# mrazomej/BarBay.jl

Measured on AMD Instinct MI355X. Metric: ELBO-grad steps/sec, 50k barcodes x 8 timepoints, higher is better.
Workload: dtype f64

## Files before the change

### barbay.jl_amd/_capi.py

```python
from __future__ import annotations

import ctypes as C
import os
from typing import Dict, List, Optional, Sequence, Tuple

import numpy as np

_HERE = os.path.dirname(os.path.abspath(__file__))
LIB_PATH = os.path.join(_HERE, "lib", "libbarbay_hip.so")

BB_MODEL = {"fitness": 0, "multienv": 1, "genotype": 2, "replicate": 3, "multienv_replicate": 4}
BB_OPT_TRUNCATED_ADAGRAD = 0
BB_OPT_DECAYED_ADAGRAD = 1
BB_COMM_ID_BYTES = 128
BB_P2P_HANDLE_BYTES = 64
BB_LOGP_MAX_BATCH = 64
BB_CHAIN_MAX_K = 16384
BB_CHAIN_MAX_Q = 8
BB_CHAIN_LAG_BATCH = 32
BB_TRACE_MAX_SNAPSHOTS = 16384
BB_SCORE_MAX_SAMPLES = 16384
BB_RB_MAX_SAMPLES = 8672
BB_RB_MAX_Q = 8
BB_THETA_RB_CHUNK = 64
BB_POPMEAN_RB_CHUNK = 256
BB_MATH_FN = {"exp": 0, "log": 1, "rcp": 2, "div": 3, "sqrt": 4, "softplus_sigmoid": 5, "sincospi": 6, "exp_nonpos": 7, "log_1to2": 8,
              "box_muller": 9}
BB_ERR_UNSUPPORTED = -4
BB_ERR_NONFINITE = -5

EXPORTS = [
    "bb_version", "bb_last_error", "bb_default_opts", "bb_create", "bb_destroy", "bb_num_latents",
    "bb_get_layout", "bb_init_meanfield", "bb_set_params", "bb_get_params", "bb_get_permutation", "bb_get_owned", "bb_run", "bb_run_profiled",
    "bb_get_posterior", "bb_elbo_grad", "bb_logdensity_grad", "bb_logdensity_grad_batch", "bb_get_elbo_trace", "bb_debug_normals", "bb_debug_math", "bb_debug_stamps", "bb_debug_graph_launches", "bb_get_stats", "bb_kernel_name",
    "bb_comm_make_id", "bb_comm_init", "bb_step_moments", "bb_step_apply", "bb_hier_units", "bb_hier_fitness", "bb_p2p_export", "bb_p2p_import", "bb_p2p_selftest", "bb_p2p_enable",
    "bb_ppc_shape", "bb_ppc_bands", "bb_freq_shape", "bb_freq_bands", "bb_score_shape", "bb_ppc_score", "bb_chain_summary",
    "bb_fitness_rb_shape", "bb_fitness_rb", "bb_theta_rb_shape", "bb_theta_rb", "bb_popmean_rb_shape", "bb_popmean_rb",
    "bb_trace_begin", "bb_trace_end", "bb_trace_count", "bb_trace_get", "bb_trace_summary",
]

_dp = C.POINTER(C.c_double)


class bb_prior(C.Structure):
    _fields_ = [("mean", _dp), ("std", _dp), ("n", C.c_int64)]


class bb_model_desc(C.Structure):
    _fields_ = [
        ("kind", C.c_int32), ("n_rep", C.c_int32), ("n_neutral", C.c_int64), ("n_bc", C.c_int64),
        ("n_time", C.POINTER(C.c_int32)), ("counts", C.POINTER(C.c_int64)), ("totals", C.POINTER(C.c_int64)),
        ("n_env", C.c_int32), ("env_idx", C.POINTER(C.c_int32)),
        ("n_geno", C.c_int32), ("geno_idx", C.POINTER(C.c_int32)),
        ("s_pop_prior", bb_prior), ("logsigma_pop_prior", bb_prior), ("s_bc_prior", bb_prior),
        ("logsigma_bc_prior", bb_prior), ("loglambda_prior", bb_prior), ("logtau_prior", bb_prior),
        ("flags", C.c_int32),
    ]


class bb_advi_opts(C.Structure):
    _fields_ = [
        ("samples_per_step", C.c_int32), ("optimizer", C.c_int32), ("eta", C.c_double), ("tau", C.c_double),
        ("window", C.c_int32), ("resum_every", C.c_int32), ("pre", C.c_double), ("post", C.c_double),
        ("seed", C.c_uint64), ("device", C.c_int32), ("rank", C.c_int32), ("world_size", C.c_int32),
        ("steps_per_graph", C.c_int32), ("elbo_every", C.c_int32), ("launch_mode", C.c_int32),
        ("n_devices", C.c_int32), ("device_ids", C.POINTER(C.c_int32)),
    ]


class bb_block_range(C.Structure):
    _fields_ = [("name", C.c_char * 24), ("lo", C.c_int64), ("hi", C.c_int64)]


class bb_stats(C.Structure):
    _fields_ = [
        ("n_latents", C.c_int64), ("n_moments", C.c_int64), ("steps_done", C.c_int64),
        ("shard_lo", C.c_int64), ("shard_hi", C.c_int64), ("bytes_per_step", C.c_int64),
        ("bytes_sample", C.c_int64), ("bytes_update", C.c_int64), ("last_run_ms", C.c_double),
        ("avg_sample_ms", C.c_double), ("avg_update_ms", C.c_double),
        ("n_blocks", C.c_int32), ("block_threads", C.c_int32), ("lds_bytes", C.c_int32),
        ("persistent_pairs", C.c_int32), ("launches_last_run", C.c_int32), ("resident_kernel", C.c_int32),
        ("geno_lo", C.c_int32), ("geno_hi", C.c_int32),
        ("device_bytes", C.c_int64), ("window_row", C.c_int64),
        ("rows_same_xcd", C.c_int32), ("reserved0", C.c_int32),
    ]


class bb_ppc_opts(C.Structure):
    _fields_ = [
        ("n_samples", C.c_int32), ("n_ppc", C.c_int32), ("n_quantiles", C.c_int32), ("reserved0", C.c_int32),
        ("quantiles", _dp), ("seed", C.c_uint64),
    ]


BB_FREQ_MODE = {"trajectory": 0, "posterior": 1}


class bb_freq_opts(C.Structure):
    _fields_ = [
        ("mode", C.c_int32), ("n_samples", C.c_int32), ("n_ppc", C.c_int32), ("n_quantiles", C.c_int32),
        ("quantiles", _dp), ("seed", C.c_uint64),
    ]


class bb_score_opts(C.Structure):
    _fields_ = [("n_samples", C.c_int32), ("reserved0", C.c_int32), ("seed", C.c_uint64)]


SCORE_CELLS = ("observed", "pred_mean", "pred_sd", "lpd", "p_waic", "pit", "pit_upper")
SCORE_ROWS = ("row_lpd", "row_p_waic")


class bb_score_out(C.Structure):
    _fields_ = [(k, _dp) for k in SCORE_CELLS + SCORE_ROWS] + [("n_scored", C.POINTER(C.c_int32))]


RB_UNITS = ("q_mean", "q_sd", "rb_mean", "rb_sd", "p_pos", "p_neg")


class bb_rb_opts(C.Structure):
    _fields_ = [("n_samples", C.c_int32), ("n_quantiles", C.c_int32), ("probs", _dp), ("threshold", C.c_double), ("seed", C.c_uint64),
                ("draws", _dp)]


class bb_rb_out(C.Structure):
    _fields_ = [(k, _dp) for k in RB_UNITS] + [("quantiles", _dp), ("n_steps", C.POINTER(C.c_int32))]


class bb_theta_rb_out(C.Structure):
    _fields_ = [(k, _dp) for k in RB_UNITS] + [("quantiles", _dp), ("n_members", C.POINTER(C.c_int32)), ("n_steps", C.POINTER(C.c_int32))]


class bb_popmean_rb_out(C.Structure):
    _fields_ = [(k, _dp) for k in RB_UNITS] + [("quantiles", _dp), ("n_members", C.POINTER(C.c_int32))]


class bb_chain_opts(C.Structure):
    _fields_ = [
        ("n_chains", C.c_int32), ("n_draws", C.c_int32), ("n_quantiles", C.c_int32), ("max_lag", C.c_int32),
        ("probs", _dp), ("slab_cols", C.c_int64),
    ]


class bb_chain_out(C.Structure):
    _fields_ = [
        ("mean", _dp), ("sd", _dp), ("mcse", _dp), ("ess", _dp), ("rhat", _dp), ("quantiles", _dp),
        ("n_lags", C.POINTER(C.c_int32)),
    ]


class bb_trace_opts(C.Structure):
    _fields_ = [("every", C.c_int32), ("capacity", C.c_int32)]


class bb_trace_sum_opts(C.Structure):
    _fields_ = [
        ("first", C.c_int64), ("n_chains", C.c_int32), ("n_draws", C.c_int32), ("max_lag", C.c_int32), ("reserved0", C.c_int32),
        ("slab_cols", C.c_int64), ("rhat_max", C.c_double),
    ]


TRACE_COLS = ("mean", "sd", "mcse", "ess", "rhat")
TRACE_BLOCK_COUNTS = ("n_cols", "n_nonfinite", "n_const", "n_above")
TRACE_BLOCK_VALUES = ("max_rhat", "min_ess", "max_mcse_rel")


class bb_trace_block(C.Structure):
    _fields_ = ([("name", C.c_char * 24), ("part", C.c_int32), ("reserved0", C.c_int32)] + [(k, C.c_int64) for k in TRACE_BLOCK_COUNTS]
                + [(k, C.c_double) for k in TRACE_BLOCK_VALUES])


class bb_trace_sum_out(C.Structure):
    _fields_ = [(k, _dp) for k in TRACE_COLS] + [("n_lags", C.POINTER(C.c_int32)), ("blocks", C.POINTER(bb_trace_block))]


class BarBayHipError(RuntimeError):
    """Raised for any non-zero status of the C ABI (the reference throws ErrorException)."""


class BarBayNonFinite(BarBayHipError):
    """bb_run took its steps but the variational parameters went NaN / Inf (BB_ERR_NONFINITE); the state can still be read."""


def _declare(lib: C.CDLL) -> C.CDLL:
    vp = C.c_void_p
    lib.bb_version.restype = C.c_char_p
    lib.bb_last_error.restype = C.c_char_p
    lib.bb_default_opts.argtypes = [C.POINTER(bb_advi_opts)]
    lib.bb_default_opts.restype = None
    lib.bb_create.argtypes = [C.POINTER(bb_model_desc), C.POINTER(bb_advi_opts), C.POINTER(vp)]
    lib.bb_destroy.argtypes = [vp]
    lib.bb_destroy.restype = None
    lib.bb_num_latents.argtypes = [vp]
    lib.bb_num_latents.restype = C.c_int64
    lib.bb_get_layout.argtypes = [vp, C.POINTER(bb_block_range), C.POINTER(C.c_int32)]
    lib.bb_init_meanfield.argtypes = [vp]
    lib.bb_set_params.argtypes = [vp, _dp, _dp]
    lib.bb_get_params.argtypes = [vp, _dp, _dp]
    if hasattr(lib, "bb_get_permutation"):
        lib.bb_get_permutation.argtypes = [vp, C.POINTER(C.c_int64)]
    if hasattr(lib, "bb_get_owned"):
        lib.bb_get_owned.argtypes = [vp, C.POINTER(C.c_int64), C.POINTER(C.c_int64)]
    lib.bb_run.argtypes = [vp, C.c_int64]
    lib.bb_run_profiled.argtypes = [vp, C.c_int64]
    lib.bb_get_posterior.argtypes = [vp, _dp, _dp]
    lib.bb_elbo_grad.argtypes = [vp, _dp, _dp, _dp, C.c_int32, _dp, _dp, _dp]
    lib.bb_logdensity_grad.argtypes = [vp, _dp, _dp, _dp]
    lib.bb_logdensity_grad_batch.argtypes = [vp, C.c_int32, _dp, _dp, _dp]
    lib.bb_get_elbo_trace.argtypes = [vp, C.c_int64, C.c_int64, _dp]
    lib.bb_debug_normals.argtypes = [vp, C.c_int64, C.c_uint32, C.c_int64, C.c_int64, _dp]
    if hasattr(lib, "bb_debug_math"):
        lib.bb_debug_math.argtypes = [vp, C.c_int32, C.c_int64, _dp, _dp, _dp, _dp]
    lib.bb_get_stats.argtypes = [vp, C.POINTER(bb_stats)]
    if hasattr(lib, "bb_kernel_name"):
        lib.bb_kernel_name.argtypes = [vp, C.c_char_p, C.c_int64]
    lib.bb_debug_stamps.argtypes = [vp, C.POINTER(C.c_uint64), C.c_int64]
    lib.bb_debug_graph_launches.argtypes = [vp]
    lib.bb_comm_make_id.argtypes = [C.c_void_p]
    lib.bb_comm_init.argtypes = [vp, C.c_void_p]
    lib.bb_step_moments.argtypes = [vp, _dp]
    lib.bb_step_apply.argtypes = [vp, _dp]
    lib.bb_p2p_export.argtypes = [vp, C.c_void_p]
    lib.bb_p2p_import.argtypes = [vp, C.c_void_p]
    lib.bb_p2p_selftest.argtypes = [vp, C.POINTER(C.c_int32)]
    lib.bb_p2p_enable.argtypes = [vp, C.c_int32]
    lib.bb_hier_units.argtypes = [vp]
    lib.bb_hier_units.restype = C.c_int64
    lib.bb_hier_fitness.argtypes = [vp, C.c_int32, C.c_uint64, _dp, _dp]
    if hasattr(lib, "bb_ppc_bands"):
        lib.bb_ppc_shape.argtypes = [vp, C.POINTER(C.c_int64), C.POINTER(C.c_int32)]
        lib.bb_ppc_bands.argtypes = [vp, C.POINTER(bb_ppc_opts), _dp, C.POINTER(C.c_int64)]
    if hasattr(lib, "bb_freq_bands"):
        lib.bb_freq_shape.argtypes = [vp, C.POINTER(C.c_int64), C.POINTER(C.c_int32)]
        lib.bb_freq_bands.argtypes = [vp, C.POINTER(bb_freq_opts), _dp, C.POINTER(C.c_int64)]
    if hasattr(lib, "bb_ppc_score"):
        lib.bb_score_shape.argtypes = [vp, C.POINTER(C.c_int64), C.POINTER(C.c_int32)]
        lib.bb_ppc_score.argtypes = [vp, C.POINTER(bb_score_opts), C.POINTER(bb_score_out)]
    if hasattr(lib, "bb_fitness_rb"):
        lib.bb_fitness_rb_shape.argtypes = [vp, C.POINTER(C.c_int64)]
        lib.bb_fitness_rb.argtypes = [vp, C.POINTER(bb_rb_opts), C.POINTER(bb_rb_out)]
    if hasattr(lib, "bb_theta_rb"):
        lib.bb_theta_rb_shape.argtypes = [vp, C.POINTER(C.c_int64)]
        lib.bb_theta_rb.argtypes = [vp, C.POINTER(bb_rb_opts), C.POINTER(bb_theta_rb_out)]
    if hasattr(lib, "bb_popmean_rb"):
        lib.bb_popmean_rb_shape.argtypes = [vp, C.POINTER(C.c_int64)]
        lib.bb_popmean_rb.argtypes = [vp, C.POINTER(bb_rb_opts), C.POINTER(bb_popmean_rb_out)]
    if hasattr(lib, "bb_chain_summary"):
        lib.bb_chain_summary.argtypes = [vp, C.POINTER(bb_chain_opts), C.c_int64, _dp, C.POINTER(bb_chain_out)]
    if hasattr(lib, "bb_trace_begin"):
        lib.bb_trace_begin.argtypes = [vp, C.POINTER(bb_trace_opts)]
        lib.bb_trace_end.argtypes = [vp]
        lib.bb_trace_count.argtypes = [vp, C.POINTER(C.c_int64), C.POINTER(C.c_int64)]
        lib.bb_trace_get.argtypes = [vp, C.c_int64, C.c_int64, _dp, _dp]
        lib.bb_trace_summary.argtypes = [vp, C.POINTER(bb_trace_sum_opts), C.POINTER(bb_trace_sum_out)]
    return lib


_LIB: Optional[C.CDLL] = None


def load_library(path: Optional[str] = None) -> C.CDLL:
    global _LIB
    if path is None and _LIB is not None:
        return _LIB
    p = path or LIB_PATH
    if not os.path.exists(p):
        raise BarBayHipError(
            f"{p} not found: build it with `python -c 'import __graft_entry__ as g; g.build()'` "
            "(hipcc --offload-arch=gfx950); there is no CPU fallback")
    try:
        import torch
    except Exception:
        pass
    lib = _declare(C.CDLL(p))
    if path is None:
        _LIB = lib
    return lib


def _f64(a) -> np.ndarray:
    return np.ascontiguousarray(a, dtype=np.float64)


def _ptr(a: np.ndarray, ty=_dp):
    return a.ctypes.data_as(ty)


class Engine:

    def __init__(self, kind: str, counts: Sequence[np.ndarray], n_neutral: int, n_bc: int, *,
                 totals: Optional[Sequence[np.ndarray]] = None, env_idx=None, geno_idx=None,
                 priors: Optional[Dict[str, Tuple[object, object]]] = None,
                 samples_per_step: int = 1, optimizer: str = "TruncatedADAGrad", eta: float = 0.1,
                 tau: float = 40.0, window: int = 100, resum_every: int = 0, pre: float = 1.0,
                 post: float = 0.9, seed: int = 0, device: int = 0, rank: int = 0, world_size: int = 1,
# ... 79 lines not shown
        return self

    def __exit__(self, *a):
        self.close()

    def layout(self) -> List[Tuple[str, int, int]]:
        blocks = (bb_block_range * 8)()
        n = C.c_int32()
        self._check(self._lib.bb_get_layout(self._h, blocks, C.byref(n)))
        return [(blocks[i].name.decode(), int(blocks[i].lo), int(blocks[i].hi)) for i in range(n.value)]

    def init_meanfield(self):
        self._check(self._lib.bb_init_meanfield(self._h))

    def set_params(self, mu, omega):
        mu, omega = _f64(mu), _f64(omega)
        assert mu.shape == (self.D,) and omega.shape == (self.D,)
        self._check(self._lib.bb_set_params(self._h, _ptr(mu), _ptr(omega)))

    def get_params(self) -> Tuple[np.ndarray, np.ndarray]:
        mu, om = np.empty(self.D), np.empty(self.D)
        self._check(self._lib.bb_get_params(self._h, _ptr(mu), _ptr(om)))
        return mu, om

    def permutation(self) -> np.ndarray:
        out = np.empty(self.D, dtype=np.int64)
        self._check(self._lib.bb_get_permutation(self._h, out.ctypes.data_as(C.POINTER(C.c_int64))))
        return out

    def owned(self) -> np.ndarray:
        out = np.empty(self.D, dtype=np.int64)
        n = C.c_int64(0)
        self._check(self._lib.bb_get_owned(self._h, out.ctypes.data_as(C.POINTER(C.c_int64)), C.byref(n)))
        return out[:n.value].copy()

    def run(self, n_steps: int):
        self._check(self._lib.bb_run(self._h, int(n_steps)))

    def run_profiled(self, n_steps: int):
        self._check(self._lib.bb_run_profiled(self._h, int(n_steps)))

    def posterior(self) -> Tuple[np.ndarray, np.ndarray]:
        m, s = np.empty(self.D), np.empty(self.D)
        self._check(self._lib.bb_get_posterior(self._h, _ptr(m), _ptr(s)))
        return m, s

    def elbo_grad(self, mu, omega, eps=None, n_samples: Optional[int] = None):
        mu, omega = _f64(mu), _f64(omega)
        if eps is not None:
            eps = np.atleast_2d(_f64(eps))
            assert eps.shape[1] == self.D
            n_samples = eps.shape[0]
        n_samples = n_samples or 1
        gm, go = np.empty(self.D), np.empty(self.D)
        elbo = C.c_double()
        self._check(self._lib.bb_elbo_grad(self._h, _ptr(mu), _ptr(omega), _ptr(eps) if eps is not None else None,
                                           n_samples, C.byref(elbo), _ptr(gm), _ptr(go)))
        return elbo.value, gm, go

    def elbo_trace(self, first_step: int, n: int) -> np.ndarray:
        out = np.empty(n)
        self._check(self._lib.bb_get_elbo_trace(self._h, first_step, n, _ptr(out)))
        return out

    def normals(self, step: int, stream: int, lo: int, hi: int) -> np.ndarray:
        out = np.empty(hi - lo)
        self._check(self._lib.bb_debug_normals(self._h, step, stream, lo, hi, _ptr(out)))
        return out

    def debug_math(self, fn, x, y=None) -> Tuple[np.ndarray, Optional[np.ndarray]]:
        code = BB_MATH_FN[fn] if isinstance(fn, str) else int(fn)
        words = code == BB_MATH_FN["box_muller"]
        x = np.ascontiguousarray(x, dtype=np.uint64).view(np.float64) if words else _f64(x)
        if y is not None:
            y = np.ascontiguousarray(y, dtype=np.uint64).view(np.float64) if words else _f64(y)
            assert y.shape == x.shape
        assert x.ndim == 1
        out0 = np.empty(x.shape[0])
        out1 = np.empty(x.shape[0]) if code in (BB_MATH_FN["softplus_sigmoid"], BB_MATH_FN["sincospi"], BB_MATH_FN["box_muller"]) else None
        self._check(self._lib.bb_debug_math(self._h, code, x.shape[0], _ptr(x), _ptr(y) if y is not None else None, _ptr(out0),
                                            _ptr(out1) if out1 is not None else None))
        return out0, out1

    def stamps(self, per_wave: bool = False) -> np.ndarray:
        nb = int(self.stats()["n_blocks"])
        rows = np.zeros(1, dtype=np.uint64)
        self._check(self._lib.bb_debug_stamps(self._h, rows.ctypes.data_as(C.POINTER(C.c_uint64)), -1))
        rows = int(rows[0])
        raw = np.zeros(rows * 96, dtype=np.uint64)
        self._check(self._lib.bb_debug_stamps(self._h, raw.ctypes.data_as(C.POINTER(C.c_uint64)), raw.size))
        if not per_wave:
            return raw[:nb * 32].reshape(nb, 32).copy()
        return raw[rows * 32:rows * 32 + nb * 64].reshape(nb, 4, 16).copy()

    def graph_launches(self) -> int:
        return int(self._lib.bb_debug_graph_launches(self._h))

    def stats(self) -> Dict[str, float]:
        s = bb_stats()
        self._check(self._lib.bb_get_stats(self._h, C.byref(s)))
        return {k: getattr(s, k) for k, _ in bb_stats._fields_}

    def kernel_name(self) -> str:
        buf = C.create_string_buffer(128)
        self._check(self._lib.bb_kernel_name(self._h, buf, 128))
        return buf.value.decode()

    def logdensity_grad(self, z) -> Tuple[float, np.ndarray]:
        z = np.ascontiguousarray(z, dtype=np.float64)
        assert z.shape == (self.D,)
        lp = C.c_double(0.0)
        g = np.empty(self.D)
        self._check(self._lib.bb_logdensity_grad(self._h, _ptr(z), C.byref(lp), _ptr(g)))
        return lp.value, g

    def logdensity_grad_batch(self, Z) -> Tuple[np.ndarray, np.ndarray]:
        Z = np.ascontiguousarray(Z, dtype=np.float64)
        if Z.ndim == 1:
            Z = Z[None, :]
        assert Z.ndim == 2 and Z.shape[1] == self.D
        W = Z.shape[0]
        lp = np.empty(W)
        g = np.empty((W, self.D))
        self._check(self._lib.bb_logdensity_grad_batch(self._h, W, _ptr(Z), _ptr(lp), _ptr(g)))
        return lp, g

    def hier_units(self) -> int:
        return int(self._lib.bb_hier_units(self._h))

    def hier_fitness(self, n_samples: int = 10_000, seed: int = 0) -> Tuple[np.ndarray, np.ndarray]:
        n = int(self._lib.bb_hier_units(self._h))
        med, sd = np.empty(n), np.empty(n)
        self._check(self._lib.bb_hier_fitness(self._h, n_samples, seed, _ptr(med), _ptr(sd)))
        return med, sd

    def ppc_shape(self) -> Tuple[int, int]:
        n, t = C.c_int64(0), C.c_int32(0)
        self._check(self._lib.bb_ppc_shape(self._h, C.byref(n), C.byref(t)))
        return int(n.value), int(t.value)

    def ppc_bands(self, quantiles: Sequence[float], n_samples: int = 1000, n_ppc: int = 10, seed: int = 0,
                  outside: bool = True) -> Tuple[np.ndarray, Optional[np.ndarray]]:
        q = _f64(np.atleast_1d(quantiles))
        n_rows, n_steps = self.ppc_shape()
        o = bb_ppc_opts()
        o.n_samples, o.n_ppc, o.n_quantiles, o.seed = int(n_samples), int(n_ppc), int(q.shape[0]), int(seed)
        o.quantiles = _ptr(q)
        bands = np.empty((n_rows, n_steps, q.shape[0], 2))
        nout = np.zeros(n_rows, dtype=np.int64) if outside else None
        self._check(self._lib.bb_ppc_bands(self._h, C.byref(o), _ptr(bands),
                                           nout.ctypes.data_as(C.POINTER(C.c_int64)) if outside else None))
        return bands, nout

    def freq_shape(self) -> Tuple[int, int]:
        n, t = C.c_int64(0), C.c_int32(0)
        self._check(self._lib.bb_freq_shape(self._h, C.byref(n), C.byref(t)))
        return int(n.value), int(t.value)

    def freq_bands(self, quantiles: Sequence[float], mode="trajectory", n_samples: int = 1000, n_ppc: int = 10, seed: int = 0,
                   outside: bool = True) -> Tuple[np.ndarray, Optional[np.ndarray]]:
        q = _f64(np.atleast_1d(quantiles))
        n_rows, n_cols = self.freq_shape()
        o = bb_freq_opts()
        o.mode = BB_FREQ_MODE[mode] if isinstance(mode, str) else int(mode)
        o.n_samples, o.n_ppc, o.n_quantiles, o.seed = int(n_samples), int(n_ppc), int(q.shape[0]), int(seed)
        o.quantiles = _ptr(q)
# ... 216 lines not shown
```

### barbay.jl_amd/csrc/bb_block.h

```cpp
#pragma once
#include "bb_types.h"
#include <math.h>
#include <string.h>

#ifdef BB_EMU
#define BB_DEV static inline
#define BB_HD static inline
struct BBCtx { int nthr; int block; double* lds; const void* lay = nullptr;  };
#define BB_PASS(cx, tid) for (int tid = 0; tid < (cx).nthr; ++tid)
#define BB_SYNC(cx) ((void)0)
BB_DEV unsigned bb_umulhi(unsigned a, unsigned b) { return (unsigned)(((unsigned long long)a * b) >> 32); }
#else
#include <hip/hip_runtime.h>
#define BB_DEV __device__ __forceinline__
#define BB_HD __host__ __device__ __forceinline__
struct BBCtx { int nthr; int block; double* lds; const void* lay = nullptr;  };
#define BB_PASS(cx, tid) for (int tid = threadIdx.x, _once = 1; _once; _once = 0)
#define BB_SYNC(cx) __syncthreads()
BB_DEV unsigned bb_umulhi(unsigned a, unsigned b) { return __umulhi(a, b); }
#endif

#if defined(BB_STAMPS) && !defined(BB_EMU)
#define BB_STAMP(cx, S, i) do { if (threadIdx.x == 0) (S).stamps[(long long)(cx).block * 32 + (i)] = __builtin_amdgcn_s_memtime(); } while (0)
#else
// ... 238 lines not shown
        e0 = a0 ? S.eps_in[(long long)A.sample * M.D + i0] : 0.0;
        e1 = a1 ? S.eps_in[(long long)A.sample * M.D + i1] : 0.0;
    } else {
        bb_normal_pair(A.seed, (unsigned long long)(i0 >> 1), step, (unsigned)A.sample, &e0, &e1);
    }
    double mu0 = 0, mu1 = 0, om0 = 0, om1 = 0;
    if (a0 && a1) {
        const bb_d2 m = *(const bb_d2*)(S.mu + i0), o = *(const bb_d2*)(S.om + i0);
        mu0 = m.x; mu1 = m.y; om0 = o.x; om1 = o.y;
    } else if (a0) { mu0 = S.mu[i0]; om0 = S.om[i0]; }
    else { mu1 = S.mu[i1]; om1 = S.om[i1]; }
    double sp0, sg0, sp1, sg1;
    bb_softplus_sigmoid(om0, &sp0, &sg0);
    bb_softplus_sigmoid(om1, &sp1, &sg1);
    *z0 = fma(sp0, e0, mu0);
    *z1 = fma(sp1, e1, mu1);
    const double h0 = sg0 * bb_rcp(sp0), h1 = sg1 * bb_rcp(sp1);
    if (a0 && a1) {
        *(bb_d2*)(S.zsv + i0) = bb_d2{*z0, *z1};
        *(bb_d2*)(S.asv + i0) = bb_d2{e0 * sg0, e1 * sg1};
        *(bb_d2*)(S.hsv + i0) = bb_d2{h0, h1};
    } else if (a0) { S.zsv[i0] = *z0; S.asv[i0] = e0 * sg0; S.hsv[i0] = h0; }
    else { S.zsv[i1] = *z1; S.asv[i1] = e1 * sg1; S.hsv[i1] = h1; }
    double el = 0.0;
    if (want_elbo) {
        const long long blo = M.blk_lo[blk];
        double pm, iv;
        if (a0) { bb_prior_of(M, blk, i0 - blo, &pm, &iv); el += -0.5 * (*z0 - pm) * (*z0 - pm) * iv + bb_log(sp0); }
        if (a1) { bb_prior_of(M, blk, i1 - blo, &pm, &iv); el += -0.5 * (*z1 - pm) * (*z1 - pm) * iv + bb_log(sp1); }
    }
    return el;
}

struct BBSlot { int slot; bool resum; };
BB_DEV BBSlot bb_slot_of(const RunArgs& A, unsigned long long step) {
    BBSlot w;
    w.slot = A.opt == 0 ? (int)(step % (unsigned long long)A.W) : 0;
    w.resum = A.opt == 0 && (A.resum_every == 1 || (A.resum_every > 1 && step > 0 && step % (unsigned long long)A.resum_every == 0));
    return w;
}

struct BBSlotCtr { int slot, rs; bool past0; };
BB_DEV int bb_uniform(int v) {
#if defined(BB_EMU)
    return v;
#else
    return __builtin_amdgcn_readfirstlane(v);
#endif
}
BB_DEV BBSlotCtr bb_slot_init(const RunArgs& A, unsigned long long step) {
    BBSlotCtr c;
    c.slot = A.opt == 0 ? bb_uniform((int)(step % (unsigned long long)A.W)) : 0;
    c.rs = (A.opt == 0 && A.resum_every > 1) ? bb_uniform((int)(step % (unsigned long long)A.resum_every)) : 0;
    c.past0 = bb_uniform(step > 0 ? 1 : 0) != 0;
    return c;
}
BB_DEV BBSlot bb_slot_now(const RunArgs& A, const BBSlotCtr& c) {
    BBSlot w;
    w.slot = c.slot;
    w.resum = A.opt == 0 && (A.resum_every == 1 || (A.resum_every > 1 && c.past0 && c.rs == 0));
    return w;
}
BB_DEV void bb_slot_next(const RunArgs& A, BBSlotCtr& c) {
    if (A.opt == 0) { c.slot = c.slot + 1 == A.W ? 0 : c.slot + 1; if (A.resum_every > 1) c.rs = c.rs + 1 == A.resum_every ? 0 : c.rs + 1; }
    c.past0 = true;
}

struct bb_f4 { float x, y, z, w; };
BB_DEV bb_f4 bb_load_lo(const DevState& S, long long i0, bool a0, bool a1) {
    bb_f4 v{0.f, 0.f, 0.f, 0.f};
    if (a0) { v.x = S.accl[2 * i0]; v.y = S.accl[2 * i0 + 1]; }
    if (a1) { v.z = S.accl[2 * i0 + 2]; v.w = S.accl[2 * i0 + 3]; }
    return v;
}
BB_DEV void bb_store_lo(const DevState& S, long long i0, bool a0, bool a1, const bb_f4& v) {
    if (a0) { S.accl[2 * i0] = v.x; S.accl[2 * i0 + 1] = v.y; }
    if (a1) { S.accl[2 * i0 + 2] = v.z; S.accl[2 * i0 + 3] = v.w; }
}
BB_DEV void bb_two_sum(double a, double b, double* s, double* e) {
    const double t = a + b, bb = t - a;
    *s = t;
    *e = (a - (t - bb)) + (b - bb);
}
BB_DEV void bb_opt_apply(const DevModel& M, const DevState& S, const RunArgs& A, const BBSlot w,
                         int which, long long ih , double d, double old_slot, double* new_slot, double* p, double* acc, float* lo) {
    double upd;
    if (A.opt == 0) {
        const double n2 = d * d;
        *new_slot = n2;
        double s;
        if (w.resum) {
            s = 0.0;
            for (int j = 0; j < A.W; ++j) s += (j == w.slot) ? n2 : S.hist[((long long)j * 2 + which) * M.Dh + ih];
            *lo = 0.f;
        } else {
            double t, e1;
            bb_two_sum(*acc, n2, &t, &e1);
            const double u = t - old_slot, e2 = (t - u) - old_slot;
            const double l = (double)*lo + (e1 + e2);
            s = u + l;
            *lo = (float)(l - (s - u));
            s = s > 0.0 ? s : 0.0;
        }
        *acc = s;
        bb_cdouble* oc = bb_tab(S.optc);
        upd = d * (oc[0] * bb_rcp(oc[1] + bb_sqrt(s)));
    } else {
        bb_cdouble* oc = bb_tab(S.optc);
        const double a = oc[3] * (*acc) + oc[2] * d * d;
        *acc = a;
        upd = d * (oc[0] * bb_rcp(bb_sqrt(a) + 1e-8));
    }
    *p -= upd;
}

BB_DEV void bb_update_pair(const DevModel& M, const DevState& S, const RunArgs& A, const BBSlot w, int blk, long long hd,
                           long long i0, bool a0, bool a1, double z0, double z1, double gl0, double gl1) {
    const long long i1 = i0 + 1, blo = M.blk_lo[blk];
    const bool both = a0 && a1;
    double pm, iv;
    double g[2] = {0.0, 0.0};
    if (a0) { bb_prior_of(M, blk, i0 - blo, &pm, &iv); g[0] = gl0 - (z0 - pm) * iv; }
    if (a1) { bb_prior_of(M, blk, i1 - blo, &pm, &iv); g[1] = gl1 - (z1 - pm) * iv; }
    bb_d2 av, hv;
    if (both) { av = *(const bb_d2*)(S.asv + i0); hv = *(const bb_d2*)(S.hsv + i0); }
    else if (a0) { av = bb_d2{S.asv[i0], 0.0}; hv = bb_d2{S.hsv[i0], 0.0}; }
    else { av = bb_d2{0.0, S.asv[i1]}; hv = bb_d2{0.0, S.hsv[i1]}; }
    double gm[2] = {g[0], g[1]}, go[2] = {g[0] * av.x, g[1] * av.y};
    if (A.S > 1) {
        const double invS = 1.0 / (double)A.S;
        for (int k = 0; k < 2; ++k) {
            if (!(k ? a1 : a0)) continue;
            const long long i = i0 + k;
            if (!A.first_sample) { gm[k] += S.gacc_mu[i]; go[k] += S.gacc_om[i]; }
            if (!A.last_sample) { S.gacc_mu[i] = gm[k]; S.gacc_om[i] = go[k]; }
            gm[k] *= invS; go[k] *= invS;
        }
        if (!A.last_sample) return;
    }
    go[0] += hv.x;
    go[1] += hv.y;
    if (!A.apply) {
        if (a0) { S.gacc_mu[i0] = gm[0]; S.gacc_om[i0] = go[0]; }
        if (a1) { S.gacc_mu[i1] = gm[1]; S.gacc_om[i1] = go[1]; }
        return;
    }
    bb_d2 mu, om, am, ao, hm = bb_d2{0, 0}, ho = bb_d2{0, 0};
    double* hs_m = nullptr;
    double* hs_o = nullptr;
    if (A.opt == 0) {
        hs_m = S.hist + ((long long)w.slot * 2 + 0) * M.Dh - hd;
        hs_o = S.hist + ((long long)w.slot * 2 + 1) * M.Dh - hd;
    }
    if (both) {
        mu = *(const bb_d2*)(S.mu + i0); om = *(const bb_d2*)(S.om + i0);
        am = *(const bb_d2*)(S.acc_mu + i0); ao = *(const bb_d2*)(S.acc_om + i0);
        if (hs_m) { hm = *(const bb_d2*)(hs_m + i0); ho = *(const bb_d2*)(hs_o + i0); }
    } else {
        const long long i = a0 ? i0 : i1;
        const double m_ = S.mu[i], o_ = S.om[i], am_ = S.acc_mu[i], ao_ = S.acc_om[i];
        const double hm_ = hs_m ? hs_m[i] : 0.0, ho_ = hs_o ? hs_o[i] : 0.0;
        mu = a0 ? bb_d2{m_, 0} : bb_d2{0, m_}; om = a0 ? bb_d2{o_, 0} : bb_d2{0, o_};
        am = a0 ? bb_d2{am_, 0} : bb_d2{0, am_}; ao = a0 ? bb_d2{ao_, 0} : bb_d2{0, ao_};
        hm = a0 ? bb_d2{hm_, 0} : bb_d2{0, hm_}; ho = a0 ? bb_d2{ho_, 0} : bb_d2{0, ho_};
    }
    bb_d2 nhm = hm, nho = ho;
    bb_f4 lo = bb_load_lo(S, i0, a0, a1);
    if (a0) {
        bb_opt_apply(M, S, A, w, 0, i0 - hd, -gm[0], hm.x, &nhm.x, &mu.x, &am.x, &lo.x);
        bb_opt_apply(M, S, A, w, 1, i0 - hd, -go[0], ho.x, &nho.x, &om.x, &ao.x, &lo.y);
    }
    if (a1) {
        bb_opt_apply(M, S, A, w, 0, i1 - hd, -gm[1], hm.y, &nhm.y, &mu.y, &am.y, &lo.z);
        bb_opt_apply(M, S, A, w, 1, i1 - hd, -go[1], ho.y, &nho.y, &om.y, &ao.y, &lo.w);
    }
    bb_store_lo(S, i0, a0, a1, lo);
    if (both) {
        *(bb_d2*)(S.mu + i0) = mu; *(bb_d2*)(S.om + i0) = om;
        *(bb_d2*)(S.acc_mu + i0) = am; *(bb_d2*)(S.acc_om + i0) = ao;
        if (hs_m) { *(bb_d2*)(hs_m + i0) = nhm; *(bb_d2*)(hs_o + i0) = nho; }
    } else {
        const long long i = a0 ? i0 : i1;
        S.mu[i] = a0 ? mu.x : mu.y; S.om[i] = a0 ? om.x : om.y;
        S.acc_mu[i] = a0 ? am.x : am.y; S.acc_om[i] = a0 ? ao.x : ao.y;
        if (hs_m) { hs_m[i] = a0 ? nhm.x : nhm.y; hs_o[i] = a0 ? nho.x : nho.y; }
    }
    const double chk = (a0 ? mu.x + om.x : 0.0) + (a1 ? mu.y + om.y : 0.0);
    if (!(chk - chk == 0.0)) S.hstatus[1] = 1u;
}
// ... 674 lines not shown
```

### barbay.jl_amd/csrc/bb_engine.hip

```cpp
#include "../../include/barbay_hip.h"
#include "bb_block.h"
#include "bb_persist.h"
#include "bb_resident.h"
#include "bb_stream.h"
#include "bb_inst.h"
#include "bb_hier.h"
#include "bb_ppc.h"
#include "bb_freq.h"
#include "bb_score.h"
#include "bb_rb.h"
#include "bb_chain.h"
#include "bb_trace.h"
#include "bb_logp.h"
#include "bb_mathprobe.h"

#include <algorithm>
#include <cmath>
#include <cstdarg>
#include <cstdio>
#include <cstdlib>
#include <cstring>
#include <ctime>
#include <string>
#include <type_traits>
#include <vector>

static thread_local char g_err[512] = "";
static int bb_fail(int code, const char* fmt, ...) {
    va_list ap;
    va_start(ap, fmt);
    vsnprintf(g_err, sizeof g_err, fmt, ap);
    va_end(ap);
    return code;
}
extern "C" const char* bb_last_error(void) { return g_err; }

#include "bb_backend.h"

extern "C" const char* bb_version(void) { return BB_BACKEND_VERSION; }

#define BB_ENTER(h) DevGuard bb_dev_guard_((h)->o.device)
#define BB_GROUP_UNSUPPORTED(h, what) \
    do { if (!(h)->shards.empty()) return bb_fail(BB_ERR_UNSUPPORTED, what " is not available on a multi-device handle (n_devices > 1)"); } while (0)

struct BBTuning {
    bool no_hist_pack, no_host_tables, no_res, no_persist, no_stream, force_stream, any_parity, force_allreduce, p2p_self;
    bool no_graph, graph_collective, no_regroup, no_reorder, nb_set, lead_set;
    int nb, res_nb, ng, lead, nthr, row_l2;
};

static BBTuning read_tuning() {
    auto set = [](const char* n) { return getenv(n) != nullptr; };
    auto num = [](const char* n, int unset) { const char* v = getenv(n); return v ? atoi(v) : unset; };
    auto on = [&](const char* n) { return num(n, 0) > 0; };
    BBTuning t{};
    t.no_hist_pack = on("BB_NO_HIST_PACK");
    t.no_host_tables = on("BB_NO_HOST_TABLES");
    t.no_res = on("BB_NO_RES");
    t.no_persist = on("BB_NO_PERSIST");
    t.no_stream = on("BB_NO_STREAM");
    t.force_stream = on("BB_TUNE_STREAM");
    t.any_parity = on("BB_TUNE_AP");
    t.force_allreduce = on("BB_FORCE_ALLREDUCE");
    t.p2p_self = on("BB_P2P_SELF");
    t.no_graph = set("BB_NO_GRAPH");
    t.graph_collective = set("BB_GRAPH_COLLECTIVE");
    t.no_regroup = set("BB_NO_REGROUP");
    t.no_reorder = set("BB_NO_REORDER");
    t.nb_set = set("BB_TUNE_NB");
    t.nb = num("BB_TUNE_NB", 0);
    t.res_nb = num("BB_TUNE_RES_NB", 0);
    t.ng = num("BB_TUNE_NG", 0);
    t.lead_set = set("BB_TUNE_LEAD");
    t.lead = num("BB_TUNE_LEAD", 65);
    if (t.lead < 10 || t.lead > 100) t.lead = 100;
    t.nthr = num("BB_TUNE_NTHR", 0) >= 64 ? num("BB_TUNE_NTHR", 0) / 64 * 64 : 0;
    t.row_l2 = num("BB_TUNE_ROW_L2", 1) == 0 ? 0 : 1;
    return t;
}

enum { IMPL_TWO_KERNEL = 0, IMPL_PERSIST = 1, IMPL_RES = 2, IMPL_STREAM = 3 };
struct LaunchPlan {
    int impl = IMPL_TWO_KERNEL;
    int P = 0;
    int NB = 0, NBL = 0, nblk = 0;
    int ng = 8, pf = 0;
    bool ms = false;
    const void* fn = nullptr;
    std::string name;
    const char* why = nullptr;
};

struct DevBuf {
    double* p = nullptr;
    size_t cap = 0;
    int grow(size_t n) {
        if (cap >= n) return 0;
        if (p) dfree(p);
        p = nullptr;
        cap = 0;
        void* q = nullptr;
        int rc = dmalloc(&q, n * 8);
        if (!rc) { p = (double*)q; cap = n; }
        return rc;
    }
};
enum {
    BUF_EPS,
    BUF_DBG,
    BUF_BANDS,
    BUF_LOGP,
    BUF_CHAIN,
    BUF_COUNT
};

struct bb_handle {
    DevModel M{};
    DevState S{};
    bb_advi_opts o{};
    std::vector<bb_block_range> blocks;
    std::vector<void*> owned;
    long long dev_bytes = 0;
    int NB = 0, nthr = 0, nblk = 0, ngeno_blk = 0;
    int tile_cap = 0;
    size_t lds_doubles = 0;
    size_t lds_doubles_p0 = 0;
    size_t lds_doubles_p = 0;
    long long b_lo = 0, b_hi = 0;
    int cus = 256;
    int g_lo = 0, g_hi = 0;
    std::vector<int> geno_ptr_h;
    long long* d_tile_b = nullptr;
    int* d_tile_g = nullptr;
    long long step = 0;
    int sample = 0;
    double elbo_const = 0.0;
    std::vector<double> ld_omega, ld_zero;
    void* p2p_inbox = nullptr;
    size_t p2p_rows_bytes = 0, p2p_bytes = 0, p2p_gran_off = 0;
    double* d_segtab = nullptr;
    int* d_ldstab = nullptr;
    size_t segtab_cap = 0, ldstab_cap = 0;
    void* p2p_peer[BB_MAX_WORLD] = {};
    bool p2p_ready = false, p2p_on = false;
    unsigned p2p_seq = 0;
    unsigned epoch0 = 0;
    long long req_steps = 0;
    bool p2p_first = false;
    unsigned* hstatus = nullptr;
    double* bak_mu = nullptr;
    double* bak_om = nullptr;
    DevBuf buf[BUF_COUNT];
    std::vector<double> logp_host;
    double* trace_ring = nullptr;
    int trace_every = 0, trace_cap = 0;
    long long trace_t = 0;
    long long trace_taken = 0;
    bbStream stream{};
    bool opened = false;
    double last_run_ms = 0, avg_sample_ms = 0, avg_update_ms = 0;
    int launches_last_run = 0;
    int graph_launches = 0;
    int64_t bytes_sample = 0, bytes_update = 0;
    BackendState be;
    BBTuning tune{};
    LaunchPlan plan;
    BRLay Yh{};
    BRLay* dY = nullptr;
    DevModel* dM = nullptr;
    DevState* dS = nullptr;
// ... 52 lines not shown
    auto cxof = [&](int b) { return BBCtx{h->nthr, b, E.lds.data() + (size_t)b * (h->lds_doubles_p + 64), &h->Lp}; };
    const BBLds L = bb_lds_layout(h->M.R, h->M.E, KIND, h->M.Ttot, h->M.nt1, h->M.K, h->NB, h->nthr, 1);
    const unsigned long long step = (unsigned long long)(h->step + it);
    const unsigned abs_epoch = A.xepoch0 + (unsigned)(step + 1), epoch = abs_epoch;
    const int par = (int)(step & 1);
    const bool xg = h->p2p_on;
    if (phase == 0) {
        for (int b = 0; b < h->nblk; ++b) {
            BBCtx cx = cxof(b);
            bbp_prologue<KIND, PP>(cx, h->M, h->S, A, h->NB, st + (size_t)b * h->nthr);
            bbp_draw_ahead<KIND, PP>(cx, h->M, A, h->NB, st + (size_t)b * h->nthr, (unsigned long long)h->step);
        }
    } else if (phase == 1) {
        for (int b = 0; b < h->nblk; ++b) {
            BBCtx cx = cxof(b);
            bbp_sample<KIND, PP>(cx, h->M, h->S, A, h->NB, st + (size_t)b * h->nthr, step);
            bbp_publish_row(cx, h->M, h->S, L, epoch);
            bbp_draw_ahead<KIND, PP>(cx, h->M, A, h->NB, st + (size_t)b * h->nthr, step + 1);
        }
    } else if (phase == 2) {
        for (int g = 0; g < bbp_groups(A); ++g) {
            BBCtx cx = cxof(g);
            if (xg) bbp_leader_reduce<true>(cx, h->M, h->S, A, L, par, epoch, &E.ok, abs_epoch);
            else bbp_leader_reduce<false>(cx, h->M, h->S, A, L, par, epoch, &E.ok, abs_epoch);
        }
    } else if (phase == 3) {
        for (int b = 0; b < h->nblk; ++b) {
            BBCtx cx = cxof(b);
            bbp_prefetch_slot<KIND, PP>(cx, h->M, h->S, A, h->NB, st + (size_t)b * h->nthr, bb_slot_of(A, step).slot);
            bbp_residual_ahead<KIND>(cx, h->M, h->NB, A);
            if (xg) bbp_consume<true>(cx, h->M, h->S, A, L, par, epoch, &E.ok, abs_epoch);
            else bbp_consume<false>(cx, h->M, h->S, A, L, par, epoch, &E.ok, abs_epoch);
            bbp_finish<KIND>(cx, h->M, h->S, A, h->NB);
            bbp_update<KIND, PP>(cx, h->M, h->S, A, h->NB, st + (size_t)b * h->nthr, bb_slot_of(A, step));
        }
    } else {
        for (int b = 0; b < h->nblk; ++b) {
            BBCtx cx = cxof(b);
            bbp_epilogue<KIND, PP>(cx, h->M, h->S, A, h->NB, st + (size_t)b * h->nthr, (unsigned long long)(h->step + nsteps), E.ok == 0);
        }
    }
}

template <int KIND, int PP, bool AP>
static void emu_res_phase(EmuPersist& E, int phase, long long it, long long nsteps) {
    bb_handle* h = E.h;
    const RunArgs& A = E.A;
    BRSt<PP>* st = (BRSt<PP>*)E.st.data();
    auto cxof = [&](int b) { return BBCtx{h->nthr, b, E.lds.data() + (size_t)b * (h->lds_doubles_p + 64), nullptr}; };
    const BRLay& Y = h->Yh;
    const int NS = A.S < 1 ? 1 : A.S;
    const bool MSrun = NS > 1 || A.elbo_every > 0;
    const unsigned long long step = (unsigned long long)(h->step + it / NS);
    const int smp = (int)(it % NS);
    const bool last = smp == NS - 1;
    const unsigned long long xc = MSrun ? step * (unsigned long long)NS + (unsigned long long)smp : step;
    const int buf = (int)(xc & 1);
    const bool want_el = MSrun && A.elbo_every > 0 && step % (unsigned long long)A.elbo_every == 0;
    const int ring = A.elbo_every > 0 ? (int)((step / (unsigned long long)A.elbo_every) % BB_ELBO_RING) : 0;
    const bool xg = h->p2p_on;
    const BBSlot wslot = bb_slot_of(A, step);
    for (int b = 0; b < (phase == 2 ? bbp_groups(A) : h->plan.nblk); ++b) {
        BBCtx cx = cxof(b);
        BRSt<PP>* sb = st + (size_t)b * h->nthr;
        if (phase == 0) {
            br_prologue<KIND, PP, AP>(cx, h->M, h->S, A, Y, h->plan.NB, sb);
            br_draw_ahead<KIND, PP, AP>(cx, A, Y, sb, (unsigned long long)h->step);
        } else if (phase == 1) {
            if (MSrun) br_sample<KIND, PP, true>(cx, h->M, h->S, A, Y, sb, buf, wslot.slot, last, want_el);
            else br_sample<KIND, PP, false>(cx, h->M, h->S, A, Y, sb, buf, wslot.slot);
            const unsigned epoch = A.xepoch0 + (unsigned)(xc + 1);
            if (MSrun) br_moments<KIND, PP, true>(cx, h->M, h->S, Y, sb, buf, epoch, want_el);
            else br_moments<KIND, PP, false>(cx, h->M, h->S, Y, sb, buf, epoch);
            br_xchg_publish<KIND, PP, AP>(cx, h->M, h->S, A, Y, sb, xc, wslot.slot, last ? step + 1 : step, last ? 0u : (unsigned)(smp + 1), last);
        } else if (phase == 2) {
            if (xg) br_xchg_lead<true>(cx, h->M, h->S, A, Y, xc, &E.ok);
            else br_xchg_lead<false>(cx, h->M, h->S, A, Y, xc, &E.ok);
        } else if (phase == 3) {
            if (xg && MSrun) br_xchg_consume<KIND, PP, true, true>(cx, h->M, h->S, A, Y, sb, xc, &E.ok, want_el, ring, smp);
            else if (xg) br_xchg_consume<KIND, PP, true, false>(cx, h->M, h->S, A, Y, sb, xc, &E.ok);
            else if (MSrun) br_xchg_consume<KIND, PP, false, true>(cx, h->M, h->S, A, Y, sb, xc, &E.ok, want_el, ring, smp);
            else br_xchg_consume<KIND, PP, false, false>(cx, h->M, h->S, A, Y, sb, xc, &E.ok);
            if (MSrun) br_update<KIND, PP, 0, AP, true>(cx, h->M, h->S, A, Y, sb, wslot, buf, h->plan.NB, smp, NS);
            else if (!AP && uniform_T(h->M) == 8) br_update<KIND, PP, 8, false>(cx, h->M, h->S, A, Y, sb, wslot, buf, h->plan.NB);
            else if (!AP && uniform_T(h->M) == 6) br_update<KIND, PP, 6, false>(cx, h->M, h->S, A, Y, sb, wslot, buf, h->plan.NB);
            else br_update<KIND, PP, 0, AP>(cx, h->M, h->S, A, Y, sb, wslot, buf, h->plan.NB);
        } else {
            br_epilogue<KIND, PP, AP>(cx, h->S, sb, (unsigned long long)(h->step + nsteps), E.ok == 0);
        }
    }
}

template <int KIND, int TT, bool MS>
static void emu_stream_phase(EmuPersist& E, int phase, long long it, long long nsteps) {
    bb_handle* h = E.h;
    const RunArgs& A = E.A;
    BSG* gs = (BSG*)E.st.data();
    auto cxof = [&](int b) { return BBCtx{h->nthr, b, E.lds.data() + (size_t)b * (h->lds_doubles_p + 64), nullptr}; };
    const BRLay& Y = h->Yh;
    const int NS = MS ? (A.S < 1 ? 1 : A.S) : 1;
    const unsigned long long step = (unsigned long long)(h->step + it / NS);
    const int smp = (int)(it % NS);
    const unsigned long long xc = step * (unsigned long long)NS + (unsigned long long)smp;
    auto rec = [&](unsigned long long st_) { return MS && A.elbo_every > 0 && st_ % (unsigned long long)A.elbo_every == 0; };
    const bool want_el = rec(step);
    const int ring = A.elbo_every > 0 ? (int)((step / (unsigned long long)A.elbo_every) % BB_ELBO_RING) : 0;
    const BSMs ms = MS ? bs_ms_of(A, step, smp, NS, want_el, rec(step + 1)) : bs_ms_plain((unsigned)step);
    BRSt<1>* nost = nullptr;
    for (int b = 0; b < (phase == 2 ? bbp_groups(A) : h->plan.nblk); ++b) {
        BBCtx cx = cxof(b);
        BSG* gb = gs + (size_t)b * h->nthr;
        int* bad_any = (int*)(cx.lds + Y.L.misc) + 3;
        if (phase == 0) {
            br_tile_setup<KIND>(cx, h->M, h->S, A, Y, h->plan.NB, KIND <= 2 ? h->nthr / 16 : h->nthr / 64);
            *bad_any = 0;
            bs_sample0<KIND, TT, MS>(cx, h->M, h->S, A, Y, h->plan.NB, h->plan.P, (unsigned)h->step, gb, (int)(((unsigned long long)h->step * (unsigned long long)NS) & 1ull), rec((unsigned long long)h->step));
        } else if (phase == 1) {
            bs_moments<KIND, TT, MS>(cx, h->M, h->S, A, Y, h->plan.NB, h->plan.P, (unsigned)step, gb, ms.buf, want_el);
            br_row_publish<1, MS>(cx, h->M, h->S, Y, nost, A.xepoch0 + (unsigned)(xc + 1), want_el);
        } else if (phase == 2) {
            br_xchg_lead<false>(cx, h->M, h->S, A, Y, xc, &E.ok);
        } else if (phase == 3) {
            br_xchg_consume<KIND, 1, false, MS>(cx, h->M, h->S, A, Y, nost, xc, &E.ok, want_el, ring, smp);
            bs_update_l<KIND, TT, MS>(cx, h->M, h->S, A, Y, h->plan.NB, h->plan.P, (unsigned)step, bb_slot_of(A, step), bad_any, gb, ms);
            bs_update_u<KIND, TT, MS>(cx, h->M, h->S, A, Y, h->plan.NB, h->plan.P, (unsigned)step, bb_slot_of(A, step), bad_any, gb, ms);
        } else {
            if (*bad_any) h->S.hstatus[1] = 1u;
            if (b == 0) { h->S.ctr[0] = (unsigned long long)(h->step + nsteps); h->S.ctr[1] = h->S.ctr[0]; }
        }
    }
}

static void emu_persist_dispatch(EmuPersist& E, int phase, long long it, long long nsteps) {
    const LaunchPlan& p = E.h->plan;
    if (p.impl == IMPL_STREAM) {
        const int T = uniform_T(E.h->M);
        auto byT = [&](auto kindc) {
            constexpr int KIND = decltype(kindc)::value;
            if (T == 8) p.ms ? emu_stream_phase<KIND, 8, true>(E, phase, it, nsteps) : emu_stream_phase<KIND, 8, false>(E, phase, it, nsteps);
            else if (T == 6) p.ms ? emu_stream_phase<KIND, 6, true>(E, phase, it, nsteps) : emu_stream_phase<KIND, 6, false>(E, phase, it, nsteps);
            else p.ms ? emu_stream_phase<KIND, 4, true>(E, phase, it, nsteps) : emu_stream_phase<KIND, 4, false>(E, phase, it, nsteps);
        };
        by_kind(E.h->M.kind, byT);
        return;
    }
    if (p.impl == IMPL_RES) {
        const bool ap = br_any_parity(E.h->M);
        auto byP = [&](auto kindc) {
            constexpr int KIND = decltype(kindc)::value;
            switch (p.P) {
            case 1: ap ? emu_res_phase<KIND, 1, true>(E, phase, it, nsteps) : emu_res_phase<KIND, 1, false>(E, phase, it, nsteps); break;
            case 2: ap ? emu_res_phase<KIND, 2, true>(E, phase, it, nsteps) : emu_res_phase<KIND, 2, false>(E, phase, it, nsteps); break;
            case 3: ap ? emu_res_phase<KIND, 3, true>(E, phase, it, nsteps) : emu_res_phase<KIND, 3, false>(E, phase, it, nsteps); break;
            default: ap ? emu_res_phase<KIND, 4, true>(E, phase, it, nsteps) : emu_res_phase<KIND, 4, false>(E, phase, it, nsteps);
            }
        };
        by_kind(E.h->M.kind, byP);
        return;
    }
    by_kind(E.h->M.kind, [&](auto kindc) {
        constexpr int KIND = decltype(kindc)::value;
        if constexpr (KIND != BB_MODEL_GENOTYPE) {
            switch (p.P) {
            case 1: emu_persist_phase<KIND, 1>(E, phase, it, nsteps); break;
            case 2: emu_persist_phase<KIND, 2>(E, phase, it, nsteps); break;
            case 3: emu_persist_phase<KIND, 3>(E, phase, it, nsteps); break;
// ... 247 lines not shown
    if (g->group_resident) {
        rc = group_run_resident(g, n_steps);
    } else {
        const int S = g->o.samples_per_step < 1 ? 1 : g->o.samples_per_step, n = (int)g->shards.size();
        std::vector<RunArgs> As((size_t)n);
        for (bb_handle* sh : g->shards) { BB_ENTER(sh); if ((rc = ensure_scratch(sh))) return rc; }
        for (int64_t it = 0; it < n_steps && !rc; ++it) {
            for (int smp = 0; smp < S && !rc; ++smp) {
                for (int i = 0; i < n; ++i) { const bb_handle* sh = g->shards[i]; As[i] = make_args(sh, sh->step, smp, S, true, elbo_wanted(sh, sh->step)); }
                rc = step_sample(g->shards.data(), n, As.data(), host_sum_exchange);
            }
            for (bb_handle* sh : g->shards) sh->step++;
        }
        for (bb_handle* sh : g->shards) { BB_ENTER(sh); const int r = dsync(sh->stream); if (r && !rc) rc = r; }
    }
    g->step = g->shards[0]->step;
    return rc;
}

static int group_get_params(bb_handle* g, double* mu, double* omega) {
    const size_t D = (size_t)g->M.D;
    std::vector<double> tm(D), to(D);
    int rc = bb_get_params(g->shards[0], mu, omega);
    for (size_t i = 1; i < g->shards.size() && !rc; ++i) {
        if ((rc = bb_get_params(g->shards[i], tm.data(), to.data()))) break;
        std::vector<std::pair<long long, long long>> rg;
        owned_ranges(g->shards[i], rg);
        for (auto& r : rg) {
            std::copy(tm.begin() + r.first, tm.begin() + r.second, mu + r.first);
            std::copy(to.begin() + r.first, to.begin() + r.second, omega + r.first);
        }
    }
    return rc;
}

extern "C" int bb_init_meanfield(bb_handle* h) {
    if (!h) return bb_fail(BB_ERR_INVALID, "null handle");
    if (!h->shards.empty()) { int rc = 0; for (bb_handle* sh : h->shards) if (!rc) rc = bb_init_meanfield(sh); h->step = 0; return rc; }
    BB_ENTER(h);
    h->theta_stale = false;
    trace_reset(h);
    const int nb = (int)std::min<long long>(((h->M.D + 1) / 2 + 255) / 256, 1024);
    const int rc = launch(h->stream, k_init, nb, 256, 0, h->M, h->S, h->o.seed);
    return rc ? rc : reset_optimizer(h);
}

extern "C" int bb_set_params(bb_handle* h, const double* mu, const double* omega) {
    if (!h || !mu || !omega) return bb_fail(BB_ERR_INVALID, "null argument");
    std::vector<double> pm, po;
    if (!h->cidx.empty()) {
        pm.resize(h->cidx.size()); po.resize(h->cidx.size());
        perm_gather(h, mu, pm.data()); perm_gather(h, omega, po.data());
        mu = pm.data(); omega = po.data();
    }
    if (!h->shards.empty()) { int rc = 0; for (bb_handle* sh : h->shards) if (!rc) rc = bb_set_params(sh, mu, omega); h->step = 0; return rc; }
    BB_ENTER(h);
    int rc;
    h->theta_stale = false;
    trace_reset(h);
    if ((rc = h2d(h->S.mu, mu, (size_t)h->M.D * 8, h->stream))) return rc;
    if ((rc = h2d(h->S.om, omega, (size_t)h->M.D * 8, h->stream))) return rc;
    return reset_optimizer(h);
}

static int get_params_raw(bb_handle* h, double* mu, double* omega) {
    if (!h->shards.empty()) return group_get_params(h, mu, omega);
    BB_ENTER(h);
    int rc;
    if ((rc = dsync(h->stream))) return rc;
    if ((rc = d2h(mu, h->S.mu, (size_t)h->M.D * 8, h->stream))) return rc;
    return d2h(omega, h->S.om, (size_t)h->M.D * 8, h->stream);
}
extern "C" int bb_get_params(bb_handle* h, double* mu, double* omega) {
    if (!h || !mu || !omega) return bb_fail(BB_ERR_INVALID, "null argument");
    if (h->cidx.empty()) return get_params_raw(h, mu, omega);
    std::vector<double> a(h->cidx.size()), b(h->cidx.size());
    int rc = get_params_raw(h, a.data(), b.data());
    if (rc) return rc;
    perm_scatter(h, a.data(), mu);
    perm_scatter(h, b.data(), omega);
    return BB_OK;
}

static double host_softplus(double om) { return std::max(om, 0.0) + log1p(exp(-fabs(om))); }

extern "C" int bb_get_posterior(bb_handle* h, double* mean, double* sigma) {
    if (!h || !mean || !sigma) return bb_fail(BB_ERR_INVALID, "null argument");
    BB_ENTER(h);
    int rc = bb_get_params(h, mean, sigma);
    if (rc) return rc;
    for (long long i = 0; i < h->M.D; ++i) sigma[i] = host_softplus(sigma[i]);
    return BB_OK;
}

extern "C" int bb_debug_normals(bb_handle* h, int64_t step, uint32_t stream, int64_t lo, int64_t hi, double* out) {
    if (!h || !out || lo < 0 || hi < lo) return bb_fail(BB_ERR_INVALID, "bad argument");
    if (!h->shards.empty()) return bb_debug_normals(h->shards[0], step, stream, lo, hi, out);
    BB_ENTER(h);
    const size_t n = (size_t)(hi - lo);
    if (n == 0) return BB_OK;
    int rc;
    DevBuf& dbg = h->buf[BUF_DBG];
    if ((rc = dbg.grow(n))) return rc;
    const int nb = (int)std::min<size_t>((n / 2 + 256) / 256, 1024);
    if ((rc = launch(h->stream, k_normals, nb, 256, 0, h->o.seed, step, stream, lo, hi, dbg.p))) return rc;
    return d2h(out, dbg.p, n * 8, h->stream);
}

extern "C" int bb_debug_math(bb_handle* h, int32_t fn, int64_t n, const double* x, const double* y, double* out0, double* out1) {
    if (!h || fn < 0 || fn >= BB_MATH_COUNT || n < 0 || !x || !out0) return bb_fail(BB_ERR_INVALID, "bad argument");
    const bool two_in = fn == BB_MATH_DIV || fn == BB_MATH_BOX_MULLER;
    const bool two_out = fn == BB_MATH_SOFTPLUS_SIGMOID || fn == BB_MATH_SINCOSPI || fn == BB_MATH_BOX_MULLER;
    if ((two_in && !y) || (two_out && !out1)) return bb_fail(BB_ERR_INVALID, "function %d takes two operands / gives two results", (int)fn);
    if (!h->shards.empty()) return bb_debug_math(h->shards[0], fn, n, x, y, out0, out1);
    BB_ENTER(h);
    if (n == 0) return BB_OK;
    const size_t m = (size_t)n;
    int rc;
    DevBuf& dbg = h->buf[BUF_DBG];
    if ((rc = dbg.grow(4 * m))) return rc;
    double *dx = dbg.p, *dy = dbg.p + m, *d0 = dbg.p + 2 * m, *d1 = dbg.p + 3 * m;
    if ((rc = h2d(dx, x, m * 8, h->stream))) return rc;
    if (two_in && (rc = h2d(dy, y, m * 8, h->stream))) return rc;
    const int nb = (int)std::min<size_t>((m + 255) / 256, 1024);
    if ((rc = launch(h->stream, k_math, nb, 256, 0, (int)fn, (long long)n, dx, two_in ? dy : nullptr, d0, two_out ? d1 : nullptr))) return rc;
    if ((rc = d2h(out0, d0, m * 8, h->stream))) return rc;
    return two_out ? d2h(out1, d1, m * 8, h->stream) : BB_OK;
}

extern "C" int bb_debug_stamps(bb_handle* h, uint64_t* out, int64_t n) {
    if (!h || !out) return bb_fail(BB_ERR_INVALID, "bad argument");
    if (!h->shards.empty()) return bb_debug_stamps(h->shards[0], out, n);
    if (n < 0) { out[0] = (uint64_t)h->tile_cap; return BB_OK; }
    BB_ENTER(h);
    const int64_t have = (int64_t)h->tile_cap * (32 + 64);
    int rc = dsync(h->stream);
    if (rc) return rc;
    return d2h(out, h->S.stamps, (size_t)std::min(n, have) * 8, h->stream);
}

extern "C" int bb_debug_graph_launches(bb_handle* h) {
    if (!h) return 0;
    if (!h->shards.empty()) return bb_debug_graph_launches(h->shards[0]);
    return h->graph_launches;
}

static size_t p2p_rows_bytes(const bb_handle* h) {
    const size_t n = (size_t)2 * h->o.world_size * 8 * (size_t)(h->M.K + 2 * h->M.nt1) * 8;
    return (n + 255) & ~(size_t)255;
}
static size_t p2p_probe_words_off(const bb_handle* h) { return (size_t)32 * 2 * h->o.world_size * 8; }

static void p2p_release(bb_handle* h) {
    for (int r = 0; r < BB_MAX_WORLD; ++r)
        if (h->p2p_peer[r] && r != h->o.rank && !h->in_group) ipc_close(h->p2p_peer[r]);
    finegrained_free(h->p2p_inbox);
    h->p2p_inbox = nullptr;
    h->p2p_ready = h->p2p_on = false;
}

static int p2p_alloc_inbox(bb_handle* h) {
    if (h->o.world_size < 2 && !h->tune.p2p_self) return bb_fail(BB_ERR_INVALID, "the cross-GPU leg needs a sharded handle (world_size > 1)");
    if (h->o.world_size > BB_MAX_WORLD) return bb_fail(BB_ERR_UNSUPPORTED, "at most %d ranks", BB_MAX_WORLD);
    if (h->M.kind == BB_MODEL_GENOTYPE && !h->M.geno_sorted)
        return bb_fail(BB_ERR_UNSUPPORTED, "the genotype model's resident launch needs geno_idx in consecutive runs (shards must own whole genotypes)");
    if (h->p2p_inbox) return BB_OK;
// ... 40 lines not shown
}

static int p2p_probe_launch(bb_handle* h, unsigned** res) {
    *res = nullptr;
    return probe_launch(h->stream, h->S, h->o.rank, h->o.world_size, p2p_probe_words_off(h), ++h->p2p_seq, res);
}
static int p2p_probe_collect(bb_handle* h, unsigned* res, int32_t* ok) {
    return probe_collect(h->stream, res, h->S, h->o.world_size, ok);
}

extern "C" int bb_p2p_selftest(bb_handle* h, int32_t* ok) {
    if (!h || !ok) return bb_fail(BB_ERR_INVALID, "null argument");
    if (!h->shards.empty()) return bb_fail(BB_ERR_UNSUPPORTED, "a multi-device handle wires its shards itself");
    BB_ENTER(h);
    *ok = 0;
    if (!h->p2p_ready) return bb_fail(BB_ERR_INVALID, "bb_p2p_import comes first");
    unsigned* res = nullptr;
    int rc = p2p_probe_launch(h, &res);
    if (rc) { probe_free(res); return rc; }
    return p2p_probe_collect(h, res, ok);
}

extern "C" int bb_p2p_enable(bb_handle* h, int32_t on) {
    if (!h) return bb_fail(BB_ERR_INVALID, "null argument");
    BB_GROUP_UNSUPPORTED(h, "bb_p2p_enable");
    BB_ENTER(h);
    if (on && !h->p2p_ready) return bb_fail(BB_ERR_INVALID, "bb_p2p_import comes first");
    Planned plan;
    int rc = plan_or_refuse(h, on ? 2 : h->o.launch_mode, on != 0, plan);
    if (rc) return rc;
    h->p2p_on = on != 0;
    if ((rc = install_plan(h, plan))) h->p2p_on = false;
    { const int rcs = sync_descriptors(h); if (!rc) rc = rcs; }
    if (rc) return rc;
    return h->p2p_on ? resident_warm(h) : BB_OK;
}

#include "bb_analysis.h"

extern "C" int bb_get_stats(bb_handle* h, bb_stats* s) {
    if (!h || !s) return bb_fail(BB_ERR_INVALID, "null argument");
    BB_ENTER(h);
    if (!h->shards.empty()) {
        int rc = bb_get_stats(h->shards[0], s);
        for (size_t i = 1; i < h->shards.size() && !rc; ++i) {
            bb_stats t;
            if ((rc = bb_get_stats(h->shards[i], &t))) break;
            s->bytes_per_step += t.bytes_per_step; s->bytes_sample += t.bytes_sample; s->bytes_update += t.bytes_update;
            s->n_blocks += t.n_blocks;
            s->rows_same_xcd += t.rows_same_xcd;
            s->device_bytes += t.device_bytes;
            s->last_run_ms = std::max(s->last_run_ms, t.last_run_ms);
            s->persistent_pairs = std::min(s->persistent_pairs, t.persistent_pairs);
            s->resident_kernel = std::min(s->resident_kernel, t.resident_kernel);
        }
        s->shard_lo = 0;
        s->shard_hi = h->M.B;
        s->geno_lo = 0;
        s->geno_hi = h->M.G;
        return rc;
    }
    memset(s, 0, sizeof *s);
    s->n_latents = h->M.D;
    s->n_moments = h->M.K;
    s->steps_done = h->step;
    s->shard_lo = h->b_lo;
    s->shard_hi = h->b_hi;
    s->geno_lo = h->g_lo;
    s->geno_hi = h->g_hi;
    s->device_bytes = h->dev_bytes;
    s->window_row = h->M.Dh;
    s->bytes_sample = h->bytes_sample;
    s->bytes_update = h->bytes_update;
    s->bytes_per_step = h->bytes_update;
    s->last_run_ms = h->last_run_ms;
    s->avg_sample_ms = h->avg_sample_ms;
    s->avg_update_ms = h->avg_update_ms;
    s->n_blocks = h->plan.nblk;
    s->block_threads = h->nthr;
    s->lds_bytes = (int32_t)((h->plan.impl != IMPL_TWO_KERNEL ? h->lds_doubles_p : h->lds_doubles) * 8);
    s->persistent_pairs = h->plan.P;
    s->launches_last_run = h->launches_last_run;
    s->resident_kernel = h->plan.impl;
    if (h->plan.impl >= IMPL_RES) {
        std::vector<int> sel((size_t)h->plan.nblk);
        int rc = d2h(sel.data(), h->S.xsel, sel.size() * sizeof(int), h->stream);
        if (rc) return rc;
        for (int v : sel) s->rows_same_xcd += v > 0 ? 1 : 0;
    }
    return BB_OK;
}

extern "C" int bb_kernel_name(bb_handle* h, char* buf, int64_t len) {
    if (!h || !buf || len < 2) return bb_fail(BB_ERR_INVALID, "null argument / no room");
    if (!h->shards.empty()) return bb_kernel_name(h->shards[0], buf, len);
    snprintf(buf, (size_t)len, "%s", h->plan.name.c_str());
    return BB_OK;
}

extern "C" int bb_comm_make_id(void* id_out) {
    if (!id_out) return bb_fail(BB_ERR_INVALID, "null argument");
    return comm_make_id(id_out);
}

extern "C" int bb_comm_init(bb_handle* h, const void* id_in) {
    if (!h || !id_in) return bb_fail(BB_ERR_INVALID, "null argument");
    BB_GROUP_UNSUPPORTED(h, "bb_comm_init");
    BB_ENTER(h);
    return comm_init(h->be, id_in, h->o.device, h->o.world_size, h->o.rank);
}
```

### barbay.jl_amd/csrc/bb_inst.h

```cpp
#pragma once
#include "bb_resident.h"
#include "bb_stream.h"

#ifndef BB_EMU
typedef void (*bb_persist_kernel)(const DevModel*, const DevState*, const BBLds*, RunArgs, int, int);
typedef void (*bb_res_kernel)(const DevModel*, const DevState*, const BRLay*, RunArgs, int, int);
#define BB_INST __attribute__((visibility("hidden")))
BB_INST bb_persist_kernel bb_persist_instance(int kind, int P, int nthr, bool xg, const char** nm = nullptr);
BB_INST bb_res_kernel bb_res_instance_k0(int P, int nthr, bool xg, int T, bool ap, bool ms, const char** nm = nullptr);
BB_INST bb_res_kernel bb_res_instance_k1(int P, int nthr, bool xg, int T, bool ap, bool ms, const char** nm = nullptr);
BB_INST bb_res_kernel bb_res_instance_k2(int P, int nthr, bool xg, int T, bool ap, bool ms, const char** nm = nullptr);
BB_INST bb_res_kernel bb_res_instance_k3(int P, int nthr, bool xg, int T, bool ap, bool ms, const char** nm = nullptr);
BB_INST bb_res_kernel bb_res_instance_k4(int P, int nthr, bool xg, int T, bool ap, bool ms, const char** nm = nullptr);
BB_INST bb_stream_kernel bb_stream_instance(int kind, int nthr, int T, const char** nm = nullptr);
BB_INST bb_stream_kernel bb_stream_instance_ms(int kind, int nthr, int T, const char** nm = nullptr);
#endif
```

### barbay.jl_amd/csrc/bb_inst_res.inc

```
#define BR_CAT2(a, b) a##b
#define BR_CAT(a, b) BR_CAT2(a, b)
#define BR_STR2(x) #x
#define BR_STR(x) BR_STR2(x)
#define BR_NM(PP, NT, XG, TT, AP, MS) "k_res<" BR_STR(BR_K) "," #PP "," #NT "," XG "," #TT "," AP "," MS ">"
#define BR_RET(PP, NT, XGb, XGs, TT, APb, APs, MSb, MSs) do { if (nm) *nm = BR_NM(PP, NT, XGs, TT, APs, MSs); return k_res<BR_K, PP, NT, XGb, TT, APb, MSb>; } while (0)
bb_res_kernel BR_CAT(bb_res_instance_k, BR_K)(int P, int nthr, bool xg, int T, bool ap, bool ms, const char** nm) {
    if (nm) *nm = "";
#define BR_T(PP, NT, TT) if (!ms && !ap && P == (PP) && T == (TT)) { if (xg) BR_RET(PP, NT, true, "true", TT, false, "false", false, "false"); BR_RET(PP, NT, false, "false", TT, false, "false", false, "false"); }
#define BR_CASE(PP, NT) case (PP): if (ms) { if (xg) { if (ap) BR_RET(PP, NT, true, "true", 0, true, "true", true, "true"); BR_RET(PP, NT, true, "true", 0, false, "false", true, "true"); } \
                                              if (ap) BR_RET(PP, NT, false, "false", 0, true, "true", true, "true"); BR_RET(PP, NT, false, "false", 0, false, "false", true, "true"); } \
                                  if (ap) { if (xg) BR_RET(PP, NT, true, "true", 0, true, "true", false, "false"); BR_RET(PP, NT, false, "false", 0, true, "true", false, "false"); } \
                                  if (xg) BR_RET(PP, NT, true, "true", 0, false, "false", false, "false"); BR_RET(PP, NT, false, "false", 0, false, "false", false, "false");
    if (nthr > 512) {
        BR_T_1024
        switch (P) { BR_P_1024 default: return nullptr; }
    }
    if (nthr > 256) {
        BR_T_512
        switch (P) { BR_CASE(1, 512) BR_CASE(2, 512) BR_CASE(3, 512) default: return nullptr; }
    }
    switch (P) { BR_CASE(1, 256) BR_CASE(2, 256) BR_CASE(3, 256) BR_CASE(4, 256) default: return nullptr; }
#undef BR_T
#undef BR_CASE
#undef BR_RET
#undef BR_NM
}
```

### barbay.jl_amd/csrc/bb_plan.h

```cpp

static int uniform_T(const DevModel& M) {
    for (int r = 1; r < M.R; ++r) if (M.T[r] != M.T[0]) return 0;
    return M.T[0];
}

static const void* resident_instance(const bb_handle* h, bool xg, bool stream, int P, bool ms, std::string& name) {
    const int kind = h->M.kind, nthr = h->nthr, T = uniform_T(h->M);
    const bool ap = br_any_parity(h->M);
#if defined(BB_EMU)
    char nm[64];
    if (stream) snprintf(nm, sizeof nm, "emu:k_stream<%d,%d,%d%s>", kind, nthr, T, ms ? ",true" : "");
    else snprintf(nm, sizeof nm, "emu:k_res<%d,%d,%d,%s,*,%s,%s>", kind, P, nthr, xg ? "true" : "false", ap ? "true" : "false", ms ? "true" : "false");
    name = nm;
    return nullptr;
#elif defined(BB_FAST_BUILD)
    name = "(experiment build)";
    if (xg || ms) return nullptr;
    auto fn = [](auto k) { return (const void*)k; };
    if (stream) {
        if (nthr == 1024 && kind == 0 && T == 8) return fn(k_stream<0, 1024, 8>);
        if (nthr == 1024 && kind == 2 && T == 8) return fn(k_stream<2, 1024, 8>);
        if (nthr == 1024 && kind == 3 && T == 6) return fn(k_stream<3, 1024, 6>);
        return nullptr;
    }
    if (ap) {
        if (nthr > 512 && P == 1 && kind == 0) return fn(k_res<0, 1, 1024, false, 0, true>);
        if (nthr > 256 && nthr <= 512 && P == 3 && kind == 3) return fn(k_res<3, 3, 512, false, 0, true>);
        return nullptr;
    }
    if (nthr > 512 && P == 1 && kind == 0) return T == 8 ? fn(k_res<0, 1, 1024, false, 8>) : fn(k_res<0, 1, 1024, false>);
    if (nthr > 512 && P == 1 && kind == 1) return T == 6 ? fn(k_res<1, 1, 1024, false, 6>) : fn(k_res<1, 1, 1024, false>);
    if (nthr > 256 && nthr <= 512 && P == 2 && kind == 0) return T == 8 ? fn(k_res<0, 2, 512, false, 8>) : fn(k_res<0, 2, 512, false>);
    if (nthr > 256 && nthr <= 512 && P == 3 && kind == 3) return T == 6 ? fn(k_res<3, 3, 512, false, 6>) : fn(k_res<3, 3, 512, false>);
    if (nthr > 256 && nthr <= 512 && P == 2 && kind == 3) return T == 6 ? fn(k_res<3, 2, 512, false, 6>) : fn(k_res<3, 2, 512, false>);
    if (nthr > 512 && P == 1 && kind == 2) return T == 8 ? fn(k_res<2, 1, 1024, false, 8>) : fn(k_res<2, 1, 1024, false>);
    return nullptr;
#else
    const char* nm = "";
    const void* k = nullptr;
    if (stream) k = ms ? (const void*)bb_stream_instance_ms(kind, nthr, T, &nm) : (const void*)bb_stream_instance(kind, nthr, T, &nm);
    else switch (kind) {
        case 0: k = (const void*)bb_res_instance_k0(P, nthr, xg, T, ap, ms, &nm); break;
        case 1: k = (const void*)bb_res_instance_k1(P, nthr, xg, T, ap, ms, &nm); break;
        case 2: k = (const void*)bb_res_instance_k2(P, nthr, xg, T, ap, ms, &nm); break;
        case 3: k = (const void*)bb_res_instance_k3(P, nthr, xg, T, ap, ms, &nm); break;
        default: k = (const void*)bb_res_instance_k4(P, nthr, xg, T, ap, ms, &nm);
    }
    name = nm;
    return k;
#endif
}
static const void* persist_instance(const bb_handle* h, bool xg, int P, std::string& name) {
#if defined(BB_EMU)
    char nm[48];
    snprintf(nm, sizeof nm, "emu:k_persist<%d,%d,%d>", h->M.kind, P, h->nthr);
    name = nm;
    return nullptr;
#elif defined(BB_FAST_BUILD)
    name = "(experiment build)";
    if (!xg && h->nthr > 512 && P == 1 && h->M.kind == 0) return (const void*)k_persist<0, 1, 1024>;
    return nullptr;
#else
    const char* nm = "";
    const void* k = (const void*)bb_persist_instance(h->M.kind, P, h->nthr, xg, &nm);
    name = nm;
    return k;
#endif
}

static long long tile_pairs_bound(const DevModel& M, long long NB) {
    long long p = 0;
    for (int r = 0; r < M.R; ++r) p += NB * M.T[r] / 2 + 1;
    if (M.kind == 0 || M.kind == 1) p += 2 * (NB * M.E / 2 + 1);
    else if (M.kind == 2) p += 3 * (NB / 2 + 1);
    else if (M.kind == 3) p += (NB / 2 + 1) + 3ll * M.R * (NB / 2 + 1);
    else p += (NB * M.E / 2 + 1) + 3ll * M.R * (NB * M.E / 2 + 1);
    p += 2 * (M.nt1 / 2 + 1);
    return p;
}

static int sync_descriptors(bb_handle* h) {
    int rc;
    if (!h->dM && ((rc = dalloc(h, &h->dM, 1)) || (rc = dalloc(h, &h->dS, 1)) || (rc = dalloc(h, &h->dL, 1)))) return rc;
    if ((rc = h2d(h->dM, &h->M, sizeof(DevModel), h->stream)) || (rc = h2d(h->dS, &h->S, sizeof(DevState), h->stream))) return rc;
    h->Lp = bb_lds_layout(h->M.R, h->M.E, h->M.kind, h->M.Ttot, h->M.nt1, h->M.K, h->NB, h->nthr, 1);
    if ((rc = h2d(h->dL, &h->Lp, sizeof(BBLds), h->stream))) return rc;
    if (!h->dY && (rc = dalloc(h, &h->dY, 1))) return rc;
    return h2d(h->dY, &h->Yh, sizeof(BRLay), h->stream);
}

struct Planned {
    LaunchPlan plan;
    bool xg = false;
    int NB0 = 0, nblk0 = 0;
    BRLay Y{};
    size_t lds_doubles = 0;
    std::vector<long long> tb;
    std::vector<int> tg;
    bool scratch = false;
    std::vector<double> segtab;
    std::vector<int> ldstab;
    int segtab_stride = 0;
};

static LaunchPlan two_kernel_plan(const bb_handle* h) {
    LaunchPlan p;
    p.NB = h->NB;
    p.nblk = h->nblk;
    p.name = step_kernels_name(h->M.kind);
    p.ms = h->o.samples_per_step != 1 || h->o.elbo_every != 0;
    return p;
}

static void base_tile_map(const bb_handle* h, Planned& c) {
    const bool nb_set = h->tune.nb_set;
    const int res_nb = h->tune.res_nb;
    const long long nbar = std::max<long long>(h->b_hi - h->b_lo, 1);
    c.NB0 = h->NB;
    c.nblk0 = h->nblk;
    if (c.nblk0 > h->cus && !nb_set) { c.NB0 = (int)((nbar + h->cus - 1) / h->cus); c.nblk0 = (int)((nbar + c.NB0 - 1) / c.NB0); }
    if (res_nb > 0) { c.NB0 = res_nb; c.nblk0 = (int)((nbar + c.NB0 - 1) / c.NB0); }
    c.plan.NB = c.NB0;
    c.plan.NBL = 0;
    c.plan.nblk = c.nblk0;
}

static bool first_hop_groups(const bb_handle* h, Planned& c) {
    const int want = h->tune.ng;
    if (h->M.K + 2 * h->M.nt1 > h->nthr) return false;
    const int KK = h->M.K + 2 * h->M.nt1;
    const bool can16 = !c.xg && c.nblk0 >= 64 && KK <= 128 && h->nthr >= 2 * (KK <= 64 ? 64 : 128);
// ... 15 lines not shown
        const double tiles = (double)c.nblk0 - (double)ng * (1.0 - pct / 100.0);
        NB = (int)std::ceil((double)nbar / tiles);
    }
    const int NBL = std::max(1, (int)(NB * (pct / 100.0)));
    const long long rest = nbar - (long long)ng * NBL;
    const int nblk = ng + (int)((std::max<long long>(rest, 0) + NB - 1) / NB);
    const long long p_uni = (br_tile_span(h->M, c.NB0, true) + h->nthr - 1) / h->nthr, p_new = (br_tile_span(h->M, NB, true) + h->nthr - 1) / h->nthr;
    if (nblk > c.nblk0 + (nb_fixed ? 8 : 0) || p_new > p_uni) return;
    c.plan.NB = NB;
    c.plan.NBL = NBL;
    c.plan.nblk = nblk;
}

static bool build_geno_tiles(const bb_handle* h, int NB, int NBL, int ng, std::vector<long long>& tb, std::vector<int>& tg) {
    const DevModel& M = h->M;
    const std::vector<int>& ptr = h->geno_ptr_h;
    auto geno_of = [&](long long m) { return (int)(std::upper_bound(ptr.begin(), ptr.end(), (int)m) - ptr.begin()) - 1; };
    auto gcut = [&](long long b) { return (b <= M.nn || b <= h->b_lo) ? h->g_lo : (b >= h->b_hi ? h->g_hi : geno_of(b - M.nn)); };
    tb.clear();
    tg.clear();
    long long b = h->b_lo;
    while (b < h->b_hi) {
        const int cap = (NBL > 0 && tb.size() < (size_t)ng) ? NBL : NB;
        long long e = std::min<long long>(b + cap, h->b_hi);
        if (e < h->b_hi && e > M.nn) {
            e = M.nn + ptr[(size_t)geno_of(e - M.nn)];
            if (e <= b) return false;
        }
        tb.push_back(b);
        tg.push_back(gcut(b));
        b = e;
    }
    if (tb.empty()) { tb.push_back(h->b_lo); tg.push_back(h->g_lo); }
    tb.push_back(h->b_hi);
    tg.push_back(h->g_hi);
    for (size_t i = 0; i + 1 < tg.size(); ++i) if (tg[i + 1] - tg[i] > NB) return false;
    return NB < 32768;
}

static bool geno_tile_table(const bb_handle* h, Planned& c) {
    const bool nb_fixed = h->tune.nb_set || h->tune.res_nb > 0;
    if (h->M.kind != BB_MODEL_GENOTYPE) return true;
    const int limit = std::max(c.nblk0, std::min(c.nblk0 + 8, h->cus));
    const int NB = c.plan.NB, NBL = c.plan.NBL, ng = c.plan.ng;
    bool ok = false;
    for (int grow = 0; grow <= NB / 2 + 8 && !ok; ++grow) {
        const int nb = NB + grow, nbl = NBL > 0 ? std::max(1, (int)((long long)NBL * nb / NB)) : 0;
        if (build_geno_tiles(h, nb, nbl, ng, c.tb, c.tg) && (int)c.tb.size() - 1 <= limit) { ok = true; c.plan.NB = nb; c.plan.NBL = nbl; }
        else if (nb_fixed && NBL > 0 && build_geno_tiles(h, nb, 0, ng, c.tb, c.tg) && (int)c.tb.size() - 1 <= limit) { ok = true; c.plan.NB = nb; c.plan.NBL = 0; }
    }
    if (!ok) return false;
    c.plan.nblk = (int)c.tb.size() - 1;
    return !(c.xg && c.plan.nblk < 8);
}

static bool pair_slots(const bb_handle* h, Planned& c) {
    const bool force_stream = h->tune.force_stream, no_stream = h->tune.no_stream;
    if (!c.xg && h->M.Dh != h->M.Dp) return false;
    c.plan.P = (int)((br_tile_span(h->M, c.plan.NB, true) + h->nthr - 1) / h->nthr);
    c.plan.impl = IMPL_RES;
    const int Pmax = h->nthr > 512 ? 2 : (h->nthr > 256 ? 3 : 4);
    if (!force_stream && c.plan.P <= Pmax) return true;
    const int T0 = uniform_T(h->M);
    const int Ps = (int)((br_tile_span(h->M, c.plan.NB, true, true) + h->nthr - 1) / h->nthr);
    if (!no_stream && !br_any_parity(h->M) && (T0 == 8 || T0 == 6 || T0 == 4) && h->nthr % 64 == 0 && !c.xg && Ps <= 64) {
        c.plan.impl = IMPL_STREAM;
        c.plan.P = Ps;
        c.scratch = h->o.samples_per_step > 1;
        return true;
    }
    return c.plan.P <= Pmax;
}

static bool window_fetch_layout(const bb_handle* h, Planned& c) {
    const bool stream = c.plan.impl == IMPL_STREAM;
    const int xrows = c.xg ? 8 * h->o.world_size : 0;
    c.plan.pf = h->o.optimizer == BB_OPT_TRUNCATED_ADAGRAD && !stream ? 1 : 0;
    c.Y = br_layout(h->M, c.plan.NB, h->nthr, c.plan.P, xrows, c.plan.pf == 1, stream);
    if (c.plan.pf != 0 && (size_t)c.Y.total * 8 > 160 * 1024) { c.plan.pf = 0; c.Y = br_layout(h->M, c.plan.NB, h->nthr, c.plan.P, xrows, false); }
    c.lds_doubles = (size_t)c.Y.total;
    return c.lds_doubles * 8 <= 160 * 1024;
}

static bool instance_fits(const bb_handle* h, Planned& c) {
    c.plan.fn = resident_instance(h, c.xg, c.plan.impl == IMPL_STREAM, c.plan.P, c.plan.ms, c.plan.name);
    if (resident_fit(c.plan.fn, h->nthr, c.lds_doubles * 8, c.plan.nblk, h->cus)) return false;
    return c.plan.nblk <= h->tile_cap;
}

template <int KIND>
static void host_tables_kind(const bb_handle* h, const RunArgs& A, const DevState& Sh, Planned& c) {
    for (int b = 0; b < A.nblk; ++b) {
        const BBTile t = KIND == 2 ? br_tile_geno(h->M, Sh, b, c.plan.NB) : br_tile(h->M, A, b, c.plan.NB);
        const int g0 = KIND == 2 ? Sh.tile_g[b] : 0, g1 = KIND == 2 ? Sh.tile_g[b + 1] : 0;
        double* rec = c.segtab.data() + (size_t)b * c.segtab_stride;
        const int n = br_build_segs<KIND>((BRSeg*)rec, h->M, c.Y, t, b == 0, g0, g1);
        ((int*)(rec + c.segtab_stride - 1))[0] = n;
    }
}
static void host_tables(const bb_handle* h, Planned& c) {
    const bool off = h->tune.no_host_tables;
    if (off) return;
    const DevModel& M = h->M;
    c.segtab_stride = BR_SEG_DOUBLES * (4 + 4 * M.R + 1) + 1;
    RunArgs A = make_args(h, 0, 0, 1, true, false);
    A.nblk = c.plan.nblk; A.nbl = c.plan.NBL; A.ng = c.plan.ng;
    DevState Sh = h->S;
    Sh.tile_b = c.tb.data();
    Sh.tile_g = c.tg.data();
    c.segtab.assign((size_t)c.plan.nblk * c.segtab_stride, 0.0);
    by_kind(M.kind, [&](auto kindc) { host_tables_kind<decltype(kindc)::value>(h, A, Sh, c); });
    const int K = M.K, Tt = M.Ttot, R = M.R;
    c.ldstab.assign((size_t)3 * K + 4 * Tt + 4 * R + 4, 0);
    for (int j = 0; j < K; ++j) br_table_row(M, c.Y, j, &c.ldstab[2 * j], &c.ldstab[2 * K + j]);
    for (int j = 0; j < Tt; ++j) br_table_time(M, c.Y.L, j, &c.ldstab[3 * K + 4 * j]);
    for (int r = 0; r < R; ++r) br_table_rep(M, c.Y, r, &c.ldstab[3 * K + 4 * Tt + 4 * r]);
}

static bool plan_resident(const bb_handle* h, bool xg, bool any_parity, Planned& out) {
    const bool no_res = h->tune.no_res;
    if (no_res || !br_eligible(h->M) || (!any_parity && br_any_parity(h->M))) return false;
    Planned c;
    c.plan = two_kernel_plan(h);
    c.xg = xg;
    base_tile_map(h, c);
    if (!first_hop_groups(h, c)) return false;
    leader_tiles(h, c);
    if (!geno_tile_table(h, c) || !pair_slots(h, c) || !window_fetch_layout(h, c) || !instance_fits(h, c)) return false;
    host_tables(h, c);
    out = std::move(c);
    return true;
}

static const char* plan_persist(const bb_handle* h, bool xg, Planned& out) {
    Planned c;
    c.plan = two_kernel_plan(h);
    c.xg = xg;
    if (c.plan.ms) return h->o.samples_per_step != 1 ? "samples_per_step != 1 and the shape has no owner-computes instance" : "ELBO recording is on and the shape has no owner-computes instance";
    if (h->M.kind == BB_MODEL_GENOTYPE)
        return h->M.geno_sorted ? "genotype model: no tile map with whole genotypes per tile fits the device" : "genotype model: geno_idx is not in consecutive runs (a tile must hold whole genotypes)";
    int P = (int)((tile_pairs_bound(h->M, h->NB) + h->nthr - 1) / h->nthr);
    if (P == 3 && h->nthr > 512) P = 4;
    if (xg && P != 1) return "sharded resident launch holds one pair per thread";
    if (P > (h->nthr > 512 ? 2 : 4)) return "tile too large for the register-resident state";
    c.lds_doubles = h->lds_doubles_p0 + (size_t)3 * P * h->nthr;
    c.plan.impl = IMPL_PERSIST;
    c.plan.P = P;
    c.plan.fn = persist_instance(h, xg, P, c.plan.name);
    if (c.lds_doubles * 8 > PERSIST_LDS_CAP) return "tile does not fit LDS with the lambda table";
    if (const char* why = resident_fit(c.plan.fn, h->nthr, c.lds_doubles * 8, h->nblk, h->cus)) return why;
    out = std::move(c);
    return nullptr;
}

static Planned plan_launch(const bb_handle* h, int mode, bool xg) {
    const bool no_persist = h->tune.no_persist, force_allreduce = h->tune.force_allreduce, any_parity = h->tune.any_parity;
    Planned c;
    c.plan = two_kernel_plan(h);
    c.xg = xg;
    if (mode == 1 || (no_persist && mode == 0)) return c;
    auto two_kernels = [&](const char* why) { c.plan.why = why; return c; };
    if (force_allreduce || (h->o.world_size != 1 && !xg)) return two_kernels("sharded run");
    if (xg && h->nblk < 8) return two_kernels("fewer than 8 tiles on this rank");
    const bool ap_first = c.plan.ms || h->M.kind == BB_MODEL_GENOTYPE || any_parity;
    Planned r;
    if (plan_resident(h, xg, ap_first, r)) return r;
    const char* why = plan_persist(h, xg, r);
    if (!why) return r;
// ... 43 lines not shown
```

### barbay.jl_amd/csrc/bb_resident.h

```cpp
#pragma once
#include "bb_persist.h"

#define BR_NCV 12
#if defined(BB_EMU) || defined(BR_NO_FENCE)
#define BR_SCHED_FENCE() ((void)0)
#else
#define BR_SCHED_FENCE() __builtin_amdgcn_sched_barrier(0)
#endif
#define BR_MAXT 16

struct BRSeg { long long lo, hi; int tbeg, span, blk, kind, ldsoff, r, lpb, T; double pm, iv; const double* mean_e; const double* iv_e; long long blo; int rstride, pad; };
#define BR_SEG_DOUBLES 12

struct BRLay {
    BBLds L;
    int zl, NBT;
    int zr0[BB_MAX_REP];
    int zlw, stw;
    int st[6], SU, nst;
    int eps;
    int hbuf;
    int racc;
    int racc_r[BB_MAX_REP], rw[BB_MAX_REP];
    int rowmap;
// ... 74 lines not shown
__host__ __device__
#endif
BRLay br_layout(const DevModel& M, int NB, int NT, int P, int xg_rows, bool own_hbuf = false, bool stream = false) {
    BRLay Y;
    const int X = (M.kind == 1) ? M.E : (M.kind == 4 ? M.E * M.R : M.R);
    const int KK = M.K + 2 * M.nt1;
    int o = 0;
    int lmax = 1;
    for (int r = 0; r < BB_MAX_REP; ++r) { Y.lpb[r] = r < M.R ? (stream ? br_lpb_stream(M.T[r]) : br_lpb(M.T[r])) : 1; if (Y.lpb[r] > lmax) lmax = Y.lpb[r]; }
    BBLds& L = Y.L;
    L = BBLds{};
    Y.NBT = 0;
    for (int r = 0; r < BB_MAX_REP; ++r) { Y.zr0[r] = Y.NBT; if (r < M.R) Y.NBT += NB * (M.T[r] + 1); }
    Y.NBT = (Y.NBT + 1) & ~1;
    if (stream) { long long sp = 0; for (int r = 0; r < M.R; ++r) sp += (long long)NB * (M.T[r] / 2); Y.NBT = (int)(2 * sp + 2); }
    {
        const BRHdr H = br_header(M.K, M.nt1, M.Ttot, M.R);
        Y.rowmap = H.rowmap; L.tmap = H.tmap; L.wk = H.wk; L.zgl = H.zgl; Y.piv = H.piv; L.invS = H.invS; L.cc = H.cc; L.GG = H.wbar; L.wbar = H.wbar;
        L.gglob = H.gglob; L.misc = H.misc; L.part = H.part; L.Dt = H.Dt; L.elbt = H.elbt; Y.iG = H.iG; Y.csum = H.csum; Y.ftab = H.ftab;
        Y.rtab = H.rtab; Y.envt = H.envt; Y.seg = H.seg; L.seg = H.seg;
        o = H.end;
    }
    Y.zlw = stream ? 1 : 2;
    Y.zl = o;      o += Y.zlw * Y.NBT;
    Y.SU = NB * X;
    Y.nst = stream ? (M.kind <= 1 ? 2 : 4) : (M.kind <= 1 ? 3 : 6);
    Y.stw = 2 * Y.SU;
    for (int i = 0; i < 6; ++i) { Y.st[i] = o; if (i < Y.nst) o += Y.stw; }
    o = (o + 1) & ~1;
    Y.gas = o;     o += stream ? (M.kind >= 2 ? Y.SU : 0) : ((M.kind == 2 || M.kind == 3) ? 2 * Y.SU : 0);
    Y.gix = o;     o += M.kind == 2 ? Y.SU + 1 : 0;
    o = (o + 1) & ~1;
    o = (o + 1) & ~1;
    Y.racc = o;
    int racc_total = 0;
    for (int r = 0; r < BB_MAX_REP; ++r) {
        Y.racc_r[r] = Y.racc + racc_total;
        Y.rw[r] = r < M.R ? (stream ? (NT / (M.R == 1 ? 16 : 64)) * Y.lpb[r] : (int)(((long long)NB * Y.lpb[r] + 63) & ~63ll)) : 0;
        if (r < M.R) racc_total += BR_NCV * (Y.rw[r] + 4);
    }
    int busy;
    if (stream) {
        Y.hbuf = Y.racc;
        busy = racc_total > 2 * Y.SU ? racc_total : 2 * Y.SU;
        o += busy;
        Y.eps = o;     o += NT / 2;
    } else if (own_hbuf) {
        Y.eps = Y.racc;
        busy = 2 * P * NT;
        o += racc_total > busy ? racc_total : busy;
        o = (o + 1) & ~1;
        Y.hbuf = o;    o += 4 * P * NT;
    } else {
        Y.hbuf = Y.racc;
        Y.eps = Y.hbuf + 4 * P * NT;
        busy = 6 * P * NT;
        o += racc_total > busy ? racc_total : busy;
    }
    { const int nch = xg_rows / 8 > 5 ? xg_rows / 8 : 5;
      L.red = o;     o += 2 * 128 + nch * ((KK + 63) & ~63) + 16; }
    (void)lmax;
    L.total = Y.total = (o + 1) & ~1;
    return Y;
}

template <int P>
struct BRSt {
    bb_d2 mu[P], om[P], am[P], ao[P];
    bb_d2 a[P], h[P];
    bb_d2 z[P];
    bb_d2 lam[P];
    long long i0[P];
    int meta[P];
    int zoff[P];
    int uo[P][3];
    int pt[P];
    int rb[P];
    int thoff[P];
    unsigned cnt[P][2];
    bb_f4 lo[P];
    bb_d2 gp[P];
    bb_d2 gm[P], go[P];
    double el;
};

enum { BRM_A0 = 1 << 4, BRM_A1 = 1 << 5, BRM_VALID = 1 << 6, BRM_MUT = 1 << 7, BRM_PREV = 1 << 8, BRM_NEXT = 1 << 9 };

template <bool AP> BB_DEV bool br_pair_aligned(long long i0) { return !AP || !(i0 & 1); }
template <bool AP> BB_DEV bb_d2 br_load_pair(const double* base, long long i0, bool a0, bool a1) {
    if (a0 && a1 && br_pair_aligned<AP>(i0)) return *(const bb_d2*)(base + i0);
    return bb_d2{a0 ? base[i0] : 0.0, a1 ? base[i0 + 1] : 0.0};
}
template <bool AP> BB_DEV void br_store_pair_stream(double* base, long long i0, bool a0, bool a1, bb_d2 v) {
#ifndef BB_EMU
    if (a0 && a1 && br_pair_aligned<AP>(i0)) {
        typedef double bb_v2d __attribute__((ext_vector_type(2)));
        bb_v2d w = {v.x, v.y};
        __builtin_nontemporal_store(w, (bb_v2d*)(base + i0));
        return;
    }
    if (a0) __builtin_nontemporal_store(v.x, base + i0);
    if (a1) __builtin_nontemporal_store(v.y, base + i0 + 1);
#else
    if (a0 && a1 && br_pair_aligned<AP>(i0)) { *(bb_d2*)(base + i0) = v; return; }
    if (a0) base[i0] = v.x;
    if (a1) base[i0 + 1] = v.y;
#endif
}
template <bool AP> BB_DEV void br_store_pair(double* base, long long i0, bool a0, bool a1, bb_d2 v) {
    if (a0 && a1 && br_pair_aligned<AP>(i0)) { *(bb_d2*)(base + i0) = v; return; }
    if (a0) base[i0] = v.x;
    if (a1) base[i0 + 1] = v.y;
}

BB_HD BBTile br_tile(const DevModel& M, const RunArgs& A, int block, int NB) {
    if (A.nbl <= 0) return bb_tile(M, A, block, NB);
    const int nlead = bbp_groups(A);
    BBTile t;
    t.NB = NB;
    const int cap = block < nlead ? A.nbl : NB;
    t.b0 = block < nlead ? A.b_lo + (long long)block * A.nbl : A.b_lo + (long long)nlead * A.nbl + (long long)(block - nlead) * NB;
    long long b1 = t.b0 + cap < A.b_hi ? t.b0 + cap : A.b_hi;
    if (t.b0 > A.b_hi) t.b0 = A.b_hi;
    t.nbt = (int)(b1 > t.b0 ? b1 - t.b0 : 0);
    long long ns = M.nn - t.b0;
    t.nshift = (int)(ns < 0 ? 0 : (ns > t.nbt ? t.nbt : ns));
    t.m0 = t.b0 + t.nshift - M.nn;
    t.nmt = t.nbt - t.nshift;
    return t;
}

BB_HD BBTile br_tile_geno(const DevModel& M, const DevState& S, int block, int NB) {
    BBTile t;
    t.NB = NB;
    t.b0 = S.tile_b[block];
    t.nbt = (int)(S.tile_b[block + 1] - t.b0);
    long long ns = M.nn - t.b0;
    t.nshift = (int)(ns < 0 ? 0 : (ns > t.nbt ? t.nbt : ns));
    t.m0 = t.b0 + t.nshift - M.nn;
    t.nmt = t.nbt - t.nshift;
    return t;
}

template <int KIND>
BB_HD int br_build_segs(BRSeg* sg, const DevModel& M, const BRLay& Y, const BBTile& t, bool globals, int g0 = 0, int g1 = 0) {
    int n = 0, cur = 0;
    auto add = [&](int blk, int kind, long long lo, long long cnt, int ldsoff, int r, int lpb, int T) {
        if (cnt <= 0) return;
        BRSeg s;
        s.lo = lo; s.hi = lo + cnt; s.blk = blk; s.kind = kind; s.ldsoff = ldsoff; s.r = r; s.lpb = lpb; s.T = T;
        s.rstride = kind == SK_L ? Y.rw[r] + 4 : 0; s.pad = (int)bb_hdelta(M, blk, r);
        s.pm = M.pri[blk].mean; s.iv = M.pri[blk].inv_var; s.mean_e = M.pri[blk].mean_e; s.iv_e = M.pri[blk].inv_var_e; s.blo = M.blk_lo[blk];
        if (kind == SK_L) { cur = (cur + 63) & ~63; s.span = (int)(cnt / T) * lpb; }
        else s.span = bb_seg_pairs(lo, lo + cnt);
        s.tbeg = cur;
        cur += s.span;
        sg[n++] = s;
    };
    for (int r = 0; r < M.R; ++r)
        add(BK_L, SK_L, M.off_l[r] + t.b0 * M.T[r], (long long)t.nbt * M.T[r], Y.zr0[r], r, Y.lpb[r], M.T[r]);
    if (KIND == 2) {
        add(BK_S, SK_TH_R, M.blk_lo[BK_S] + g0, g1 - g0, 0, 0, 0, 0);
        add(BK_TT, SK_TT_R, M.blk_lo[BK_TT] + t.m0, t.nmt, 0, 0, 0, M.T[0]);
        add(BK_LT, SK_LT_R, M.blk_lo[BK_LT] + t.m0, t.nmt, 0, 0, 0, M.T[0]);
        add(BK_LS, SK_LS_R, M.blk_lo[BK_LS] + t.m0, t.nmt, 0, 0, 0, M.T[0]);
    } else if (t.nmt > 0) {
// ... 192 lines not shown
    }
    BB_STAMP_RT(cx, S, 9);
}

template <int KIND, int P, bool AP = false>
BB_DEV void br_prologue(BBCtx& cx, const DevModel& M, const DevState& S, const RunArgs& A, const BRLay& Y, int NB, BRSt<P>* stv) {
    double* lds = cx.lds;
    const BBLds& L = Y.L;
    const BBTile t = KIND == 2 ? br_tile_geno(M, S, cx.block, NB) : br_tile(M, A, cx.block, NB);
    const int g0 = KIND == 2 ? S.tile_g[cx.block] : 0, g1 = KIND == 2 ? S.tile_g[cx.block + 1] : 0;
    const BRSeg* sg = (const BRSeg*)(lds + Y.seg);
    const int* li = (const int*)(lds + L.misc);
    br_tile_setup<KIND>(cx, M, S, A, Y, NB, -1);
    BB_PASS(cx, tid) {
        const int nseg = li[0];
        BRSt<P>& st = BB_PSTATE(stv, tid);
#pragma unroll
        for (int k = 0; k < P; ++k) {
            br_desc<KIND, P, AP>(M, Y, t, sg, nseg, g0, g1, tid + k * cx.nthr, st, k, lds);
            const long long i0 = st.i0[k];
            const int meta = st.meta[k];
            const bool a0 = meta & BRM_A0, a1 = meta & BRM_A1;
            st.mu[k] = br_load_pair<AP>(S.mu, i0, a0, a1);
            st.om[k] = br_load_pair<AP>(S.om, i0, a0, a1);
            st.am[k] = br_load_pair<AP>(S.acc_mu, i0, a0, a1);
            st.ao[k] = br_load_pair<AP>(S.acc_om, i0, a0, a1);
            st.lo[k] = bb_load_lo(S, i0, a0, a1);
            st.a[k] = st.h[k] = st.z[k] = st.lam[k] = st.gp[k] = bb_d2{0.0, 0.0};
        }
    }
    BB_STAMP_RT(cx, S, 10);
    BB_SYNC(cx);
}

template <int P> struct BRIdx { long long i0[P]; int meta[P]; };

template <int P, bool MAYODD>
#ifdef BB_EMU
static inline
#else
__device__ __attribute__((noinline))
#endif
void br_draw_call(bb_d2* eps, int nthr, int tid, unsigned long long seed, unsigned step, unsigned stream,
                  long long i0a, long long i0b, long long i0c, long long i0d, int ma, int mb, int mc, int md) {
    BRIdx<P> ix;
    { const long long i0v[4] = {i0a, i0b, i0c, i0d}; const int mv[4] = {ma, mb, mc, md};
#pragma unroll
      for (int k = 0; k < P; ++k) { ix.i0[k] = i0v[k]; ix.meta[k] = mv[k]; } }
#pragma unroll
    for (int k = 0; k < P; ++k) {
        if (!(ix.meta[k] & BRM_VALID)) continue;
        const bool odd = MAYODD && (ix.i0[k] & 1);
        double e0 = 0.0, e1 = 0.0;
#pragma nounroll
        for (int rep = 0; rep < (odd ? 2 : 1); ++rep) {
            double a, b;
            bb_normal_pair(seed, (unsigned long long)(ix.i0[k] >> 1) + (unsigned long long)rep, step, stream, &a, &b);
            if (rep == 0) { e0 = odd ? b : a; e1 = b; }
            else e1 = a;
        }
        eps[k * nthr + tid] = bb_d2{e0, e1};
    }
}

template <int KIND, int P, bool AP = false>
BB_DEV void br_draw_ahead(BBCtx& cx, const RunArgs& A, const BRLay& Y, BRSt<P>* stv, unsigned long long step, unsigned stream = 0u) {
    bb_d2* eps = (bb_d2*)(cx.lds + Y.eps);
    BB_PASS(cx, tid) {
        BRSt<P>& st = BB_PSTATE(stv, tid);
        static_assert(P <= 4, "br_draw_call takes four pair slots");
        br_draw_call<P, AP>(eps, cx.nthr, tid, A.seed, (unsigned)step, stream, st.i0[0], P > 1 ? st.i0[P > 1 ? 1 : 0] : 0, P > 2 ? st.i0[P > 2 ? 2 : 0] : 0,
                            P > 3 ? st.i0[P > 3 ? 3 : 0] : 0, st.meta[0], P > 1 ? st.meta[P > 1 ? 1 : 0] : 0, P > 2 ? st.meta[P > 2 ? 2 : 0] : 0, P > 3 ? st.meta[P > 3 ? 3 : 0] : 0);
    }
}

template <int KIND> BB_DEV int br_stage_raw(int kind) {
    if (KIND <= 1) return kind == SK_S ? 0 : 2;
    return kind == SK_TH_R ? 3 : (kind == SK_TT_R ? 0 : (kind == SK_LT_R ? 4 : 5));
}
template <int KIND> BB_DEV int br_stage_trn(int kind) {
    if (KIND <= 1) return kind == SK_LS_E ? 1 : -1;
    return kind == SK_LT_R ? 1 : (kind == SK_LS_R ? 2 : -1);
}
template <int KIND>
BB_DEV void br_unit_sw(const double* lds, const BRLay& Y, int buf, int o, int thoff, double* s, double* w) {
    const double* b = lds + buf * Y.SU;
    if (KIND <= 1) { *s = b[BR_ST(Y, 0) + o]; *w = b[BR_ST(Y, 1) + o]; }
    else { *s = fma(b[BR_ST(Y, 1) + o], b[BR_ST(Y, 0) + o], b[BR_ST(Y, 3) + o - thoff]); *w = b[BR_ST(Y, 2) + o]; }
}

#ifdef BB_EMU
#define BR_HDELTA(HD, lds, Y, meta) (((const BRSeg*)((lds) + (Y).seg))[(meta) >> 12].pad)
#else
#define BR_HDELTA(HD, lds, Y, meta) ((HD) ? ((const BRSeg*)((lds) + (Y).seg))[(meta) >> 12].pad : 0)
#endif
template <int P, bool HD = false>
BB_DEV void br_prefetch_slot(BBCtx& cx, const DevModel& M, const DevState& S, const RunArgs& A, const BRLay& Y, BRSt<P>* stv, int slot);
template <int KIND, int P> BB_DEV void br_pair_prior(const double* lds, const BRLay& Y, const BRSt<P>& st, int k, bool a0, bool a1, double* pm0, double* iv0, double* pm1, double* iv1);
template <int KIND, int P, bool MS = false, bool HD = false>
BB_DEV void br_sample(BBCtx& cx, const DevModel& M, const DevState& S, const RunArgs& A, const BRLay& Y, BRSt<P>* stv, int buf, int slot, bool prefetch = true, bool want_el = false) {
    double* lds = cx.lds;
    const BBLds& L = Y.L;
    BB_STAMP(cx, S, 20);
    BB_STAMP_WAVE(cx, S, A, 1);
    if (A.pf == 1 && prefetch) br_prefetch_slot<P, HD>(cx, M, S, A, Y, stv, slot);
    BB_PASS(cx, tid) {
        BRSt<P>& st = BB_PSTATE(stv, tid);
#pragma unroll
        for (int k = 0; k < P; ++k) {
#ifdef BB_EMU
            if (!(st.meta[k] & BRM_VALID)) continue;
#else
            if (P > 1 && __builtin_amdgcn_ballot_w64((st.meta[k] & BRM_VALID) != 0) == 0ull) continue;
#endif
            const bb_d2 e = ((const bb_d2*)(lds + Y.eps))[k * cx.nthr + tid];
            double sp0, sg0, sp1, sg1;
            bb_softplus_sigmoid(st.om[k].x, &sp0, &sg0);
            bb_softplus_sigmoid(st.om[k].y, &sp1, &sg1);
            st.z[k] = bb_d2{fma(sp0, e.x, st.mu[k].x), fma(sp1, e.y, st.mu[k].y)};
            st.a[k] = bb_d2{e.x * sg0, e.y * sg1};
            st.h[k] = bb_d2{sg0 * bb_rcp(sp0), sg1 * bb_rcp(sp1)};
            if (MS && want_el) {
                if (k == 0) st.el = 0.0;
                const int meta = st.meta[k], kd = meta & 15;
                const bool counted = (meta & BRM_VALID) && (kd < SK_GS || A.count_globals);
                if (counted) {
                    const bool a0 = meta & BRM_A0, a1 = meta & BRM_A1;
                    double pm0, iv0, pm1, iv1;
                    br_pair_prior<KIND>(lds, Y, st, k, a0, a1, &pm0, &iv0, &pm1, &iv1);
                    if (a0) st.el += -0.5 * (st.z[k].x - pm0) * (st.z[k].x - pm0) * iv0 + bb_log(sp0);
                    if (a1) st.el += -0.5 * (st.z[k].y - pm1) * (st.z[k].y - pm1) * iv1 + bb_log(sp1);
                }
            }
            BR_SCHED_FENCE();
            const int kd = st.meta[k] & 15;
            const double f = (kd == SK_LS_E || (KIND >= 2 && kd == SK_LS_R)) ? -2.0 : 1.0;
#ifndef BB_EMU
            if (__builtin_amdgcn_ballot_w64((st.meta[k] & BRM_VALID) && (kd == SK_L || (kd < SK_GS && br_stage_trn<KIND>(kd) >= 0))) == 0ull) st.lam[k] = bb_d2{0.0, 0.0};
            else
#endif
            st.lam[k] = bb_d2{bb_exp(f * st.z[k].x), bb_exp(f * st.z[k].y)};
            BR_SCHED_FENCE();
            if (MS && want_el && (st.meta[k] & BRM_VALID)) {
                const int meta = st.meta[k];
                if (kd == SK_L) {
                    st.el += (double)st.cnt[k][0] * st.z[k].x - st.lam[k].x;
                    if (meta & BRM_A1) st.el += (double)st.cnt[k][1] * st.z[k].y - st.lam[k].y;
                } else if (kd == SK_LS_E || (KIND >= 2 && kd == SK_LS_R)) {
                    const BRSeg* sgk = (const BRSeg*)(lds + Y.seg) + (meta >> 12);
                    const int T1 = sgk->T - 1;
#pragma unroll
                    for (int x = 0; x < 2; ++x) {
                        if (!(meta & (x ? BRM_A1 : BRM_A0))) continue;
                        int n = T1;
                        if (KIND == 1 || KIND == 4) {
                            const int* envt = (const int*)(lds + Y.envt);
                            const int e_ = (st.uo[k][2] >> (8 * x)) & 255, tc = KIND == 4 ? M.tcum[st.pt[k]] : 0;
                            n = 0;
                            for (int tt = 0; tt < T1; ++tt) n += envt[tc + tt + 1] == e_ ? 1 : 0;
                        }
                        st.el -= (x ? st.z[k].y : st.z[k].x) * (double)n;
                    }
                }
            }
        }
#pragma unroll
        for (int k = 0; k < P; ++k) {
            const int meta = st.meta[k];
            if (!(meta & BRM_VALID)) continue;
            const int kind = meta & 15;
            if (kind == SK_L) {
                double* zw = lds + Y.zl + buf * Y.NBT + st.zoff[k];
                zw[0] = st.z[k].x;
                zw[1] = st.z[k].y;
            } else if (kind < SK_GS) {
                const int raw = br_stage_raw<KIND>(kind), trn = br_stage_trn<KIND>(kind);
                double* dst = lds + BR_ST(Y, raw) + buf * Y.SU + st.zoff[k];
                if (meta & BRM_A0) dst[0] = st.z[k].x;
                if (meta & BRM_A1) dst[1] = st.z[k].y;
                if (trn >= 0) {
                    double* dw = lds + BR_ST(Y, trn) + buf * Y.SU + st.zoff[k];
                    if (meta & BRM_A0) dw[0] = st.lam[k].x;
                    if (meta & BRM_A1) dw[1] = st.lam[k].y;
                }
            } else {
                double* dst = lds + L.wk + M.K + (kind == SK_GLS ? M.nt1 : 0) + st.zoff[k];
                if (A.count_globals) {
                    if (meta & BRM_A0) dst[0] = st.z[k].x;
                    if (meta & BRM_A1) dst[1] = st.z[k].y;
                }
            }
        }
    }
    BB_STAMP_WAVE(cx, S, A, 0);
    BB_SYNC(cx);
    BB_STAMP(cx, S, 21);
}

#ifndef BB_EMU
template <int CTRL>
__device__ __forceinline__ double br_dpp(double x) {
    int lo = __double2loint(x), hi = __double2hiint(x);
    lo = __builtin_amdgcn_update_dpp(0, lo, CTRL, 0xF, 0xF, false);
    hi = __builtin_amdgcn_update_dpp(0, hi, CTRL, 0xF, 0xF, false);
    return __hiloint2double(hi, lo);
}
__device__ __forceinline__ double br_row16_sum(double s) {
    s += br_dpp<0x128>(s);
    s += br_dpp<0x124>(s);
    s += br_dpp<0x122>(s);
    s += br_dpp<0x121>(s);
    return s;
}
#endif

template <int P, bool MS = false>
BB_DEV void br_row_publish(BBCtx& cx, const DevModel& M, const DevState& S, const BRLay& Y, BRSt<P>* stv, unsigned epoch, bool want_el = false) {
    double* lds = cx.lds;
    BB_STAMP(cx, S, 23);
    const int KK = M.K + 2 * M.nt1, KS = bb_row_stride(KK);
    const int* rm = (const int*)(lds + Y.rowmap);
// ... 145 lines not shown
            const int* ft = (const int*)(lds + Y.ftab) + 4 * j;
            const int mo = ft[0], zo = ft[1], hasprev = ft[2];
            double Dt = 0.0, c = 0.0, wb = 0.0;
            if (mo >= 0) {
                const double nn = (double)M.nn;
                const double* mm = lds + mo;
                const double M0 = mm[0], M1 = mm[1], N1 = mm[3], N2 = mm[4];
                const double sbar = lds[L.zgl + zo], ls = lds[L.zgl + M.nt1 + zo];
                wb = bb_exp(-2.0 * ls);
                const double dl = bb_log(lds[ft[3] + 1] * lds[L.invS + j]);
                const double cp = (dl - lds[Y.piv + j]) - sbar;
                c = dl - sbar;
                const double quadN = N2 - 2.0 * cp * N1 + nn * cp * cp;
                Dt = (M1 - cp * M0) + wb * (N1 - cp * nn);
                lds[L.gglob + zo] = -Dt;
                lds[L.gglob + M.nt1 + zo] = wb * quadN - nn;
                if (MS && want_el) {
                    const double M2 = mm[2], quadM = M2 - 2.0 * cp * M1 + cp * cp * M0;
                    lds[L.elbt + j] = -0.5 * (quadM + wb * quadN) - nn * ls;
                }
            } else if (MS && want_el) lds[L.elbt + j] = 0.0;
            lds[L.cc + j] = c;
            lds[L.wbar + j] = wb;
            lds[L.Dt + j] = Dt;
            lds[Y.iG + j] = ((hasprev ? lds[L.Dt + j - 1] : 0.0) - Dt) * lds[L.invS + j];
        }
    }
    BB_SYNC(cx);
    BB_STAMP(cx, S, 26);
    if (MS && want_el && cx.block == 0) {
        BB_PASS(cx, tid) {
            if (tid == 0) {
                const RunArgs& A = *Ap;
                double v = lds[L.wk + M.K - 2] + lds[L.wk + M.K - 1] + A.elbo_const;
                for (int j = 0; j < M.Ttot; ++j) v += lds[L.elbt + j];
                double* slot = S.elbo_ring + ring;
                *slot = (smp == 0 ? 0.0 : *slot) + v / (double)A.S;
            }
        }
    }
}

template <int KIND, int P>
BB_DEV void br_pair_prior(const double* lds, const BRLay& Y, const BRSt<P>& st, int k, bool a0, bool a1, double* pm0, double* iv0, double* pm1, double* iv1) {
    const BRSeg* sgk = (const BRSeg*)(lds + Y.seg) + (st.meta[k] >> 12);
    *pm0 = *pm1 = sgk->pm;
    *iv0 = *iv1 = sgk->iv;
    if (sgk->mean_e) {
        const long long j = st.i0[k] - sgk->blo;
        if (a0) { *pm0 = sgk->mean_e[j]; *iv0 = sgk->iv_e[j]; }
        if (a1) { *pm1 = sgk->mean_e[j + 1]; *iv1 = sgk->iv_e[j + 1]; }
    }
}
template <int KIND, int P>
BB_DEV void br_pair_diffs(const double* lds, const BRLay& Y, const BRSt<P>& st, int k, int buf, double* z0, double* z1,
                          double* ap, double* am, double* an, double* wp, double* wm, double* wn) {
    const int meta = st.meta[k];
    const bool hp = meta & BRM_PREV, hn = meta & BRM_NEXT;
    const double* zb = lds + Y.zl + buf * Y.NBT + st.zoff[k];
    *z0 = zb[0]; *z1 = zb[1];
    const double zp = hp ? zb[-1] : *z0, zn = hn ? zb[2] : *z1;
    *ap = *z0 - zp; *am = *z1 - *z0; *an = zn - *z1;
    *wp = *wm = *wn = 0.0;
    if (meta & BRM_MUT) {
        double sp, sm, sn;
        br_unit_sw<KIND>(lds, Y, buf, st.uo[k][1], KIND >= 2 ? st.thoff[k] : 0, &sm, wm);
        if (KIND == 1 || KIND == 4) {
            br_unit_sw<KIND>(lds, Y, buf, st.uo[k][0], KIND >= 3 ? st.thoff[k] : 0, &sp, wp);
            br_unit_sw<KIND>(lds, Y, buf, st.uo[k][2], KIND >= 3 ? st.thoff[k] : 0, &sn, wn);
        } else { sp = sn = sm; *wp = *wn = *wm; }
        *ap -= sp; *am -= sm; *an -= sn;
    }
}
template <int KIND, int P> BB_DEV constexpr bool br_has_pre() { return P == 1 && KIND <= 1; }
template <int KIND, int P, bool AP = false>
BB_DEV void br_grad_pre(BBCtx& cx, const BRLay& Y, BRSt<P>* stv, int buf) {
    if (!br_has_pre<KIND, P>()) return;
    const double* lds = cx.lds;
    BB_PASS(cx, tid) {
        BRSt<P>& st = BB_PSTATE(stv, tid);
#pragma unroll
        for (int k = 0; k < P; ++k) {
            const int meta = st.meta[k];
            if ((meta & 15) != SK_L || !(meta & BRM_VALID)) continue;
            const bool hp = meta & BRM_PREV, hn = meta & BRM_NEXT;
            double pm0, iv0, pm1, iv1, z0, z1, ap, am, an, wp, wm, wn;
            br_pair_prior<KIND>(lds, Y, st, k, true, AP ? (st.meta[k] & BRM_A1) != 0 : true, &pm0, &iv0, &pm1, &iv1);
            br_pair_diffs<KIND>(lds, Y, st, k, buf, &z0, &z1, &ap, &am, &an, &wp, &wm, &wn);
            double A0 = ((double)st.cnt[k][0] - st.lam[k].x) - (z0 - pm0) * iv0;
            double A1 = ((double)st.cnt[k][1] - st.lam[k].y) - (z1 - pm1) * iv1;
            if (meta & BRM_MUT) {
                const double ma = (AP && !(meta & BRM_A1)) ? 0.0 : wm * am;
                A0 += ma - (hp ? wp * ap : 0.0);
                A1 += (hn ? wn * an : 0.0) - ma;
            }
            st.gp[k] = bb_d2{A0, A1};
        }
    }
}
template <int KIND, int P, int TT>
BB_DEV void br_theta_pre(BBCtx& cx, const DevModel& M, const BRLay& Y, BRSt<P>* stv, int buf) {
    if (KIND != 2 && KIND != 3) return;
    double* lds = cx.lds;
    BB_PASS(cx, tid) {
        BRSt<P>& st = BB_PSTATE(stv, tid);
#pragma unroll
        for (int k = 0; k < P; ++k) {
            const int meta = st.meta[k];
            if ((meta & 15) != SK_TT_R || !(meta & BRM_VALID)) continue;
            const int* rt = (const int*)(lds + Y.rtab) + 4 * (KIND == 2 ? 0 : st.pt[k]);
            const int T = TT ? TT : rt[2];
            const double* zbuf = lds + Y.zl + buf * Y.NBT + (KIND == 2 ? Y.zr0[0] : rt[1]);
#pragma unroll
            for (int x = 0; x < 2; ++x) {
                if (!(meta & (x ? BRM_A1 : BRM_A0))) continue;
                const int j = st.zoff[k] + x, bl = st.uo[k][x];
                const int th = KIND == 2 ? j - ((st.uo[k][2] >> (16 * x)) & 0xffff) : st.thoff[k];
                double sv, wv;
                br_unit_sw<KIND>(lds, Y, buf, j, th, &sv, &wv);
                const double* zr = zbuf + bl * (T + 1);
                *(bb_d2*)(lds + Y.gas + 2 * j) = bb_d2{wv * ((zr[T - 1] - zr[0]) - (double)(T - 1) * sv), wv};
            }
        }
    }
}

template <int KIND, int P>
BB_DEV void br_theta_sum(BBCtx& cx, const DevModel& M, const BRLay& Y, BRSt<P>* stv) {
    if (KIND != 2) return;
    const double* lds = cx.lds;
    BB_PASS(cx, tid) {
        BRSt<P>& st = BB_PSTATE(stv, tid);
#pragma unroll
        for (int k = 0; k < P; ++k) {
            const int meta = st.meta[k];
            if ((meta & 15) != SK_TH_R || !(meta & BRM_VALID)) continue;
            bb_d2 sa{0.0, 0.0}, sw{0.0, 0.0};
#pragma unroll
            for (int x = 0; x < 2; ++x) {
                if (!(meta & (x ? BRM_A1 : BRM_A0))) continue;
                const int first = st.uo[k][x] & 0xffff, n = st.uo[k][x] >> 16;
                const bb_d2* ge = (const bb_d2*)(lds + Y.gas) + first;
                double a = 0.0, w = 0.0;
                int i = 0;
                for (; i + 4 <= n; i += 4) {
                    const bb_d2 e0 = ge[i], e1 = ge[i + 1], e2 = ge[i + 2], e3 = ge[i + 3];
                    a += (e0.x + e1.x) + (e2.x + e3.x);
                    w += (e0.y + e1.y) + (e2.y + e3.y);
                }
                for (; i < n; ++i) { a += ge[i].x; w += ge[i].y; }
                if (x) { sa.y = a; sw.y = w; } else { sa.x = a; sw.x = w; }
            }
            st.gp[k] = sa;
            st.lam[k] = sw;
        }
    }
}

template <int KIND, int P, bool AP = false, bool PRE = (P == 1 && KIND <= 1)>
BB_DEV void br_l_grad(const double* lds, const BRLay& Y, const BRSt<P>& st, int k, int buf, double* g0, double* g1) {
    const BBLds& L = Y.L;
    const int meta = st.meta[k], pt = st.pt[k];
    const bool hp = meta & BRM_PREV, hn = meta & BRM_NEXT;
    const double cp = hp ? lds[L.cc + pt - 1] : 0.0, cm = lds[L.cc + pt], cn = hn ? lds[L.cc + pt + 1] : 0.0;
    if (!PRE) {
        double pm0, iv0, pm1, iv1, z0, z1, ap, am, an, wp, wm, wn;
        br_pair_prior<KIND>(lds, Y, st, k, true, AP ? (st.meta[k] & BRM_A1) != 0 : true, &pm0, &iv0, &pm1, &iv1);
        br_pair_diffs<KIND>(lds, Y, st, k, buf, &z0, &z1, &ap, &am, &an, &wp, &wm, &wn);
        if (!(meta & BRM_MUT)) { wp = hp ? lds[L.wbar + pt - 1] : 0.0; wm = lds[L.wbar + pt]; wn = lds[L.wbar + pt + 1]; }
        const double rp_ = hp ? wp * (ap - cp) : 0.0, rm_ = (AP && !(meta & BRM_A1)) ? 0.0 : wm * (am - cm), rn_ = hn ? wn * (an - cn) : 0.0;
        const double l0 = st.lam[k].x, l1 = st.lam[k].y;
        *g0 = ((double)st.cnt[k][0] - l0) + l0 * lds[Y.iG + pt] + rm_ - rp_ - (z0 - pm0) * iv0;
        *g1 = ((double)st.cnt[k][1] - l1) + l1 * lds[Y.iG + pt + 1] + rn_ - rm_ - (z1 - pm1) * iv1;
        return;
    }
    double rp, rm, rn;
    if (meta & BRM_MUT) {
        double s_, wp, wm, wn;
        br_unit_sw<KIND>(lds, Y, buf, st.uo[k][1], KIND >= 2 ? st.thoff[k] : 0, &s_, &wm);
        if (KIND == 1 || KIND == 4) {
            br_unit_sw<KIND>(lds, Y, buf, st.uo[k][0], KIND >= 3 ? st.thoff[k] : 0, &s_, &wp);
            br_unit_sw<KIND>(lds, Y, buf, st.uo[k][2], KIND >= 3 ? st.thoff[k] : 0, &s_, &wn);
        } else { wp = wn = wm; }
        rp = -(wp * cp); rm = -(wm * cm); rn = -(wn * cn);
    } else {
        double z0, z1, ap, am, an, wp, wm, wn;
        br_pair_diffs<KIND>(lds, Y, st, k, buf, &z0, &z1, &ap, &am, &an, &wp, &wm, &wn);
        rp = hp ? lds[L.wbar + pt - 1] * (ap - cp) : 0.0;
        rm = (AP && !(meta & BRM_A1)) ? 0.0 : lds[L.wbar + pt] * (am - cm);
        rn = hn ? lds[L.wbar + pt + 1] * (an - cn) : 0.0;
    }
    *g0 = fma(st.lam[k].x, lds[Y.iG + pt], st.gp[k].x) + (rm - rp);
    *g1 = fma(st.lam[k].y, lds[Y.iG + pt + 1], st.gp[k].y) + (rn - rm);
}

template <int KIND, int P, int TT = 0, bool AP = false, bool MS = false, bool HD = false>
BB_DEV void br_update(BBCtx& cx, const DevModel& M, const DevState& S, const RunArgs& A, const BRLay& Y, BRSt<P>* stv,
                      const BBSlot wslot, int buf, int NBs, int smp = 0, int NS = 1) {
    double* lds = cx.lds;
    const BBLds& L = Y.L;
    BB_STAMP_WAVE(cx, S, A, 2);
#ifndef BB_EMU
    {
        bool u = false;
#pragma unroll
        for (int k = 0; k < P; ++k) u = u || ((stv->meta[k] & BRM_VALID) && (stv->meta[k] & 15) != SK_L);
        if (__builtin_amdgcn_ballot_w64(u) != 0ull) __builtin_amdgcn_s_setprio(3);
    }
#endif
    const double* zbuf = lds + Y.zl + buf * Y.NBT;
    BB_PASS(cx, tid) {
        BRSt<P>& st = BB_PSTATE(stv, tid);
        double* hs_m = nullptr;
        double* hs_o = nullptr;
        if (A.opt == 0) {
            hs_m = S.hist + ((long long)wslot.slot * 2 + 0) * M.Dh;
            hs_o = S.hist + ((long long)wslot.slot * 2 + 1) * M.Dh;
        }
#pragma unroll
        for (int k = 0; k < P; ++k) {
            const int meta = st.meta[k];
            if (!(meta & BRM_VALID)) continue;
            const int kind = meta & 15;
            const bool a0 = meta & BRM_A0, a1 = meta & BRM_A1;
            double pm0 = 0.0, pm1 = 0.0, iv0 = 0.0, iv1 = 0.0;
            if (kind != SK_L) br_pair_prior<KIND>(lds, Y, st, k, a0, a1, &pm0, &iv0, &pm1, &iv1);
            double g0 = 0.0, g1 = 0.0, z0 = 0.0, z1 = 0.0;
            if (kind == SK_L) {
                br_l_grad<KIND, P, AP>(lds, Y, st, k, buf, &g0, &g1);
            } else if (KIND == 2 && kind == SK_TH_R) {
                const double* stg = lds + buf * Y.SU;
                double csum = 0.0;
                { const int T = TT ? TT : M.T[0]; for (int tt = 0; tt < T - 1; ++tt) csum += lds[L.cc + tt]; }
#pragma unroll
                for (int x = 0; x < 2; ++x) {
                    if (!(x ? a1 : a0)) continue;
                    (x ? g1 : g0) = (x ? st.gp[k].y : st.gp[k].x) - (x ? st.lam[k].y : st.lam[k].x) * csum;
                    (x ? z1 : z0) = stg[BR_ST(Y, 3) + st.zoff[k] + x];
                }
            } else if (kind < SK_GS) {
                const int* envt = (const int*)(lds + Y.envt);
                const double* stg = lds + buf * Y.SU;
                const int E = (KIND == 1 || KIND == 4) ? M.E : 1;
                double gx[2] = {0.0, 0.0}, zx[2] = {0.0, 0.0};
#pragma unroll
                for (int x = 0; x < 2; ++x) {
                    if (!(x ? a1 : a0)) continue;
                    const int j = st.zoff[k] + x;
                    const int e = KIND == 2 ? 0 : (st.uo[k][2] >> (8 * x)) & 255, bl = st.uo[k][x];
                    zx[x] = stg[BR_ST(Y, br_stage_raw<KIND>(kind)) + j];
                    const bool is_th = KIND >= 3 && kind == SK_TH_R;
                    if (KIND == 3 && is_th) {
                        double acc = 0.0;
                        for (int r = 0; r < M.R; ++r) {
                            const int* rt = (const int*)(lds + Y.rtab) + 4 * r;
                            const int T = TT ? TT : rt[2];
                            double csum = 0.0;
                            for (int tt = 0; tt < T - 1; ++tt) csum += lds[L.cc + rt[0] + tt];
                            const bb_d2 ge = *(const bb_d2*)(lds + Y.gas + 2 * (r * NBs + j));
                            acc += ge.x - ge.y * csum;
                        }
                        gx[x] = acc;
                        continue;
                    }
                    const int r0 = KIND <= 1 ? 0 : (is_th ? 0 : st.pt[k]), r1 = KIND <= 1 ? 1 : (is_th ? M.R : r0 + 1);
                    double acc = 0.0;
                    for (int r = r0; r < r1; ++r) {
                        const int o = is_th ? (r * NBs + (j / E)) * E + e : j;
                        const int th = KIND <= 1 ? 0 : (KIND == 2 ? j - ((st.uo[k][2] >> (16 * x)) & 0xffff) : (is_th ? r * NBs * E : st.thoff[k]));
                        double sv, wv;
                        br_unit_sw<KIND>(lds, Y, buf, o, th, &sv, &wv);
                        const int* rt = (const int*)(lds + Y.rtab) + 4 * r;
                        const int T = TT ? TT : rt[2], tc = KIND <= 1 ? 0 : rt[0];
                        const double* zr = zbuf + (KIND <= 1 ? Y.zr0[0] : rt[1]) + bl * (T + 1);
                        double As = 0.0, Qs = 0.0;
                        int nn = 0;
                        if (TT) {
                            double zrow[TT ? TT : 1];
#pragma unroll
                            for (int tt = 0; tt < TT; ++tt) zrow[tt] = zr[tt];
#pragma unroll
                            for (int tt = 0; tt < TT - 1; ++tt) {
                                const bool use = E == 1 || envt[tc + tt + 1] == e;
                                const double rr = use ? (zrow[tt + 1] - zrow[tt]) - sv - lds[L.cc + tc + tt] : 0.0;
                                As += rr; Qs += rr * rr; nn += use ? 1 : 0;
                            }
                        } else {
                            for (int tt = 0; tt < T - 1; ++tt) {
                                if (E > 1 && envt[tc + tt + 1] != e) continue;
                                const double rr = (zr[tt + 1] - zr[tt]) - sv - lds[L.cc + tc + tt];
                                As += rr; Qs += rr * rr; ++nn;
                            }
                        }
                        if (KIND <= 1) acc = kind == SK_S ? wv * As : wv * Qs - (double)nn;
                        else if (is_th) acc += wv * As;
                        else if (kind == SK_LS_R) acc = wv * Qs - (double)nn;
                        else if (kind == SK_TT_R) acc = wv * As * stg[BR_ST(Y, 1) + j];
                        else acc = wv * As * stg[BR_ST(Y, 1) + j] * stg[BR_ST(Y, 0) + j];
                    }
                    gx[x] = acc;
                }
                g0 = gx[0]; g1 = gx[1]; z0 = zx[0]; z1 = zx[1];
            } else {
                const double* gg = lds + L.gglob + (kind == SK_GLS ? M.nt1 : 0) + st.zoff[k];
                const double* zz = lds + L.zgl + (kind == SK_GLS ? M.nt1 : 0) + st.zoff[k];
                if (a0) { g0 = gg[0]; z0 = zz[0]; }
                if (a1) { g1 = gg[1]; z1 = zz[1]; }
            }
            g0 -= (z0 - pm0) * iv0;
            g1 -= (z1 - pm1) * iv1;
            double go0, go1;
            if (MS && NS > 1) {
                go0 = g0 * st.a[k].x; go1 = g1 * st.a[k].y;
                if (smp > 0) { g0 += st.gm[k].x; g1 += st.gm[k].y; go0 += st.go[k].x; go1 += st.go[k].y; }
                if (smp < NS - 1) { st.gm[k] = bb_d2{g0, g1}; st.go[k] = bb_d2{go0, go1}; continue; }
                const double invS = 1.0 / (double)NS;
                g0 *= invS; g1 *= invS;
                go0 = go0 * invS + st.h[k].x; go1 = go1 * invS + st.h[k].y;
            } else { go0 = fma(g0, st.a[k].x, st.h[k].x); go1 = fma(g1, st.a[k].y, st.h[k].y); }
            bb_d2 hm{0, 0}, ho{0, 0};
            if (hs_m) {
#ifndef BB_EMU
                asm volatile("s_waitcnt vmcnt(0)" ::: "memory");
#endif
                hm = ((const bb_d2*)(lds + Y.hbuf))[(k * 2 + 0) * cx.nthr + tid];
                ho = ((const bb_d2*)(lds + Y.hbuf))[(k * 2 + 1) * cx.nthr + tid];
            }
            bb_d2 nhm = hm, nho = ho;
            const long long ih = st.i0[k] - BR_HDELTA(HD, lds, Y, meta);
            if (a0) {
                bb_opt_apply(M, S, A, wslot, 0, ih, -g0, hm.x, &nhm.x, &st.mu[k].x, &st.am[k].x, &st.lo[k].x);
                BR_SCHED_FENCE();
                bb_opt_apply(M, S, A, wslot, 1, ih, -go0, ho.x, &nho.x, &st.om[k].x, &st.ao[k].x, &st.lo[k].y);
                BR_SCHED_FENCE();
            }
            if (a1) {
                bb_opt_apply(M, S, A, wslot, 0, ih + 1, -g1, hm.y, &nhm.y, &st.mu[k].y, &st.am[k].y, &st.lo[k].z);
                BR_SCHED_FENCE();
                bb_opt_apply(M, S, A, wslot, 1, ih + 1, -go1, ho.y, &nho.y, &st.om[k].y, &st.ao[k].y, &st.lo[k].w);
                BR_SCHED_FENCE();
            }
            if (hs_m) { br_store_pair_stream<AP>(hs_m, ih, a0, a1, nhm); br_store_pair_stream<AP>(hs_o, ih, a0, a1, nho); }
        }
    }
#ifndef BB_EMU
    __builtin_amdgcn_s_setprio(0);
#endif
    BB_STAMP_WAVE(cx, S, A, 3);
    BB_STAMP(cx, S, 28);
}

template <int KIND, int P, bool AP = false>
BB_DEV void br_epilogue(BBCtx& cx, const DevState& S, BRSt<P>* stv, unsigned long long step_end, bool timed_out) {
    BB_PASS(cx, tid) {
        BRSt<P>& st = BB_PSTATE(stv, tid);
        bool bad = false;
#pragma unroll
        for (int k = 0; k < P; ++k) {
            const int meta = st.meta[k];
            if (!(meta & BRM_VALID)) continue;
            const bool a0 = meta & BRM_A0, a1 = meta & BRM_A1;
            br_store_pair<AP>(S.mu, st.i0[k], a0, a1, st.mu[k]);
            br_store_pair<AP>(S.om, st.i0[k], a0, a1, st.om[k]);
            br_store_pair<AP>(S.acc_mu, st.i0[k], a0, a1, st.am[k]);
            br_store_pair<AP>(S.acc_om, st.i0[k], a0, a1, st.ao[k]);
            bb_store_lo(S, st.i0[k], a0, a1, st.lo[k]);
            const double chk = (a0 ? st.mu[k].x + st.om[k].x : 0.0) + (a1 ? st.mu[k].y + st.om[k].y : 0.0);
            bad = bad || !(chk - chk == 0.0);
        }
        if (bad) S.hstatus[1] = 1u;
        if (timed_out && tid == 0) S.hstatus[0] = 1u;
        if (cx.block == 0 && tid == 0) { S.ctr[0] = step_end; S.ctr[1] = step_end; }
    }
    BB_SYNC(cx);
}

template <int KIND, int P, bool AP = false, bool HD = false>
BB_DEV void br_xchg_publish(BBCtx& cx, const DevModel& M, const DevState& S, const RunArgs& A, const BRLay& Y, BRSt<P>* stv, unsigned long long xc, int slot,
                            unsigned long long next_step, unsigned next_stream = 0u, bool prefetch = true) {
    if (A.pf == 0 && prefetch) br_prefetch_slot<P, HD>(cx, M, S, A, Y, stv, slot);
    br_grad_pre<KIND, P, AP>(cx, Y, stv, (int)(xc & 1));
    br_theta_sum<KIND, P>(cx, M, Y, stv);
    if (KIND == 3) br_theta_pre<KIND, P, 0>(cx, M, Y, stv, (int)(xc & 1));
    br_draw_ahead<KIND, P, AP>(cx, A, Y, stv, next_step, next_stream);
}
template <bool XG>
BB_DEV void br_xchg_lead(BBCtx& cx, const DevModel& M, const DevState& S, const RunArgs& A, const BRLay& Y, unsigned long long xc, int* ok_slot) {
    const unsigned epoch = A.xepoch0 + (unsigned)(xc + 1);
    if (cx.block < bbp_groups(A)) bbp_leader_reduce_tg<XG>(cx, M, S, A, Y.L, (int)(xc & 1), epoch, ok_slot);
}
template <int KIND, int P, bool XG, bool MS = false>
BB_DEV void br_xchg_consume(BBCtx& cx, const DevModel& M, const DevState& S, const RunArgs& A, const BRLay& Y, BRSt<P>* stv,
                            unsigned long long xc, int* ok_slot, bool want_el = false, int ring = 0, int smp = 0) {
    const unsigned epoch = A.xepoch0 + (unsigned)(xc + 1);
    if (XG) bbp_consume_tgx(cx, M, S, A, Y.L, (int)(xc & 1), epoch, ok_slot);
    else bbp_consume_tg(cx, M, S, A, Y.L, (int)(xc & 1), epoch, ok_slot);
    br_finish<KIND, MS>(cx, M, S, Y, &A, want_el, ring, smp);
}

#ifndef BB_EMU
template <int KIND, int P, int NT, bool XG = false, int TT = 0, bool AP = false, bool MS = false>
__global__ void __launch_bounds__(NT) k_res(const DevModel* __restrict__ Mp, const DevState* __restrict__ Sp, const BRLay* __restrict__ Yp,
                                            RunArgs A, int NB, int nsteps) {
    const DevModel& M = *Mp;
    const DevState& S = *Sp;
    const BRLay& Y = *Yp;
    extern __shared__ __attribute__((aligned(16))) double br_smem[];
    BBCtx cx{(int)blockDim.x, (int)blockIdx.x, br_smem, nullptr};
    BRSt<P> st;
    int* ok_slot = (int*)(br_smem + Yp->L.misc) + 1;
    const unsigned long long c0 = S.ctr[0], c1 = S.ctr[1];
    unsigned long long step0 = c0 > c1 ? c0 : c1;
    step0 = ((unsigned long long)(unsigned)__builtin_amdgcn_readfirstlane((int)(step0 >> 32)) << 32) | (unsigned)__builtin_amdgcn_readfirstlane((int)step0);
    BB_STAMP_RT(cx, S, 2);
    br_prologue<KIND, P, AP>(cx, M, S, A, Y, NB, &st);
    BB_STAMP_RT(cx, S, 3);
    const bool dead = *ok_slot == 0;
    int done = 0;
    if (!dead) {
        br_draw_ahead<KIND, P, AP>(cx, A, Y, &st, step0);
        BB_STAMP_RT(cx, S, 4);
        BBSlotCtr sc = bb_slot_init(A, step0);
        const int NS = MS ? A.S : 1;
        int ec = (MS && A.elbo_every > 0) ? bb_uniform((int)(step0 % (unsigned long long)A.elbo_every)) : 1;
        int ring = (MS && A.elbo_every > 0) ? bb_uniform((int)(((step0 + (unsigned long long)A.elbo_every - 1ull) / (unsigned long long)A.elbo_every) % BB_ELBO_RING)) : 0;
        for (; done < nsteps; ++done, bb_slot_next(A, sc)) {
            const unsigned long long step = step0 + (unsigned long long)done;
            const BBSlot wslot = bb_slot_now(A, sc);
            const bool want_el = MS && A.elbo_every > 0 && ec == 0;
            bool stop = false;
            for (int smp = 0; smp < NS; ++smp) {
                const unsigned long long xc = MS ? step * (unsigned long long)NS + (unsigned long long)smp : step;
                const int buf = (int)(xc & 1);
                const bool last = smp == NS - 1;
                if (P > 1 || KIND >= 2) {
#pragma unroll
                    for (int k = 0; k < P; ++k) asm volatile("" : "+v"(st.meta[k]));
                }
                br_sample<KIND, P, MS, XG>(cx, M, S, A, Y, &st, buf, wslot.slot, last, want_el);
                br_moments<KIND, P, MS>(cx, M, S, Y, &st, buf, A.xepoch0 + (unsigned)(xc + 1), want_el);
                br_xchg_publish<KIND, P, AP, XG>(cx, M, S, A, Y, &st, xc, wslot.slot, last ? step + 1 : step, last ? 0u : (unsigned)(smp + 1), last);
                br_xchg_lead<XG>(cx, M, S, A, Y, xc, ok_slot);
                br_xchg_consume<KIND, P, XG, MS>(cx, M, S, A, Y, &st, xc, ok_slot, want_el, ring, smp);
                if (*ok_slot == 0) { stop = true; break; }
                br_update<KIND, P, TT, AP, MS, XG>(cx, M, S, A, Y, &st, wslot, buf, NB, smp, NS);
            }
            if (stop) break;
            if (MS && A.elbo_every > 0) {
                if (ec == 0) ring = ring + 1 == BB_ELBO_RING ? 0 : ring + 1;
                ec = ec + 1 == A.elbo_every ? 0 : ec + 1;
            }
        }
    }
    BB_STAMP_RT(cx, S, 5);
    asm volatile("s_waitcnt vmcnt(0)" ::: "memory");
    br_epilogue<KIND, P, AP>(cx, S, &st, step0 + (unsigned long long)done, dead || *ok_slot == 0);
    BB_STAMP_RT(cx, S, 6);
}
#endif
```

### include/barbay_hip.h

```cpp
#ifndef BARBAY_HIP_H
#define BARBAY_HIP_H

#include <stdint.h>

#ifdef __cplusplus
extern "C" {
#endif

#define BB_OK 0
#define BB_ERR_INVALID (-1)
#define BB_ERR_DEVICE (-2)
#define BB_ERR_COMM (-3)
#define BB_ERR_UNSUPPORTED (-4)
#define BB_ERR_NONFINITE (-5)

#define BB_MODEL_FITNESS 0
#define BB_MODEL_MULTIENV 1
#define BB_MODEL_GENOTYPE 2
#define BB_MODEL_REPLICATE 3

#define BB_MODEL_MULTIENV_REPLICATE 4

#define BB_FLAG_RAGGED_METHOD 1

#define BB_OPT_TRUNCATED_ADAGRAD 0
#define BB_OPT_DECAYED_ADAGRAD 1

typedef struct bb_prior {
    const double* mean;
    const double* std;
    int64_t n;
} bb_prior;

typedef struct bb_model_desc {
    int32_t kind;
    int32_t n_rep;
    int64_t n_neutral;
    int64_t n_bc;
    const int32_t* n_time;
    const int64_t* counts;
    const int64_t* totals;
    int32_t n_env;
    const int32_t* env_idx;
    int32_t n_geno;
    const int32_t* geno_idx;
    bb_prior s_pop_prior;
    bb_prior logsigma_pop_prior;
    bb_prior s_bc_prior;
    bb_prior logsigma_bc_prior;
    bb_prior loglambda_prior;
    bb_prior logtau_prior;
    int32_t flags;
} bb_model_desc;

typedef struct bb_advi_opts {
    int32_t samples_per_step;
    int32_t optimizer;
    double eta;
    double tau;
    int32_t window;
    int32_t resum_every;
    double pre;
    double post;
    uint64_t seed;
    int32_t device;
    int32_t rank;
    int32_t world_size;
    int32_t steps_per_graph;
    int32_t elbo_every;
    int32_t launch_mode;
    int32_t n_devices;
    const int32_t* device_ids;
} bb_advi_opts;

typedef struct bb_handle bb_handle;

typedef struct bb_block_range {
    char name[24];
    int64_t lo;
    int64_t hi;
} bb_block_range;

typedef struct bb_stats {
    int64_t n_latents;
    int64_t n_moments;
    int64_t steps_done;
    int64_t shard_lo, shard_hi;
    int64_t bytes_per_step;
    int64_t bytes_sample, bytes_update;
    double last_run_ms;
    double avg_sample_ms;
    double avg_update_ms;
    int32_t n_blocks, block_threads, lds_bytes;
    int32_t persistent_pairs;
    int32_t launches_last_run;
    int32_t resident_kernel;
    int32_t geno_lo, geno_hi;
    int64_t device_bytes;
    int64_t window_row;
    int32_t rows_same_xcd;
    int32_t reserved0;
} bb_stats;

const char* bb_version(void);
const char* bb_last_error(void);

void bb_default_opts(bb_advi_opts* opts);

int bb_create(const bb_model_desc* model, const bb_advi_opts* opts, bb_handle** out);
void bb_destroy(bb_handle* h);

int64_t bb_num_latents(const bb_handle* h);
int bb_get_layout(const bb_handle* h, bb_block_range* blocks, int32_t* n_blocks);

int bb_init_meanfield(bb_handle* h);
int bb_set_params(bb_handle* h, const double* mu, const double* omega);
int bb_get_params(bb_handle* h, double* mu, double* omega);
int bb_get_permutation(bb_handle* h, int64_t* caller_index);
int bb_get_owned(bb_handle* h, int64_t* idx, int64_t* n);

int bb_run(bb_handle* h, int64_t n_steps);
int bb_run_profiled(bb_handle* h, int64_t n_steps);

int bb_get_posterior(bb_handle* h, double* mean, double* sigma);

int bb_elbo_grad(bb_handle* h, const double* mu, const double* omega, const double* eps,
                 int32_t n_samples, double* elbo, double* grad_mu, double* grad_omega);

#define BB_P2P_HANDLE_BYTES 64
int bb_p2p_export(bb_handle* h, void* handle_out);
int bb_p2p_import(bb_handle* h, const void* handles);
int bb_p2p_selftest(bb_handle* h, int32_t* ok);
int bb_p2p_enable(bb_handle* h, int32_t on);

int bb_logdensity_grad(bb_handle* h, const double* z, double* logp, double* grad);

#define BB_LOGP_MAX_BATCH 64
int bb_logdensity_grad_batch(bb_handle* h, int32_t n_points, const double* z ,
                             double* logp , double* grad );

int bb_get_elbo_trace(bb_handle* h, int64_t first_step, int64_t n, double* out);

int64_t bb_hier_units(const bb_handle* h);
int bb_hier_fitness(bb_handle* h, int32_t n_samples, uint64_t seed, double* median, double* std);

typedef struct bb_ppc_opts {
    int32_t n_samples;
    int32_t n_ppc;
    int32_t n_quantiles;
    int32_t reserved0;
    const double* quantiles;
    uint64_t seed;
} bb_ppc_opts;
int bb_ppc_shape(const bb_handle* h, int64_t* n_rows, int32_t* n_steps);
int bb_ppc_bands(bb_handle* h, const bb_ppc_opts* o, double* bands ,
                 int64_t* n_outside );

#define BB_FREQ_TRAJECTORY 0
#define BB_FREQ_POSTERIOR 1
typedef struct bb_freq_opts {
    int32_t mode;
    int32_t n_samples;
    int32_t n_ppc;
    int32_t n_quantiles;
    const double* quantiles;
    uint64_t seed;
} bb_freq_opts;
int bb_freq_shape(const bb_handle* h, int64_t* n_rows, int32_t* n_cols);
int bb_freq_bands(bb_handle* h, const bb_freq_opts* o, double* bands ,
                  int64_t* n_outside );

#define BB_SCORE_MAX_SAMPLES 16384
typedef struct bb_score_opts {
    int32_t n_samples;
    int32_t reserved0;
    uint64_t seed;
} bb_score_opts;
typedef struct bb_score_out {
    double *observed, *pred_mean, *pred_sd, *lpd, *p_waic, *pit, *pit_upper;
    double *row_lpd, *row_p_waic;
    int32_t* n_scored;
} bb_score_out;
int bb_score_shape(const bb_handle* h, int64_t* n_rows, int32_t* n_steps);
int bb_ppc_score(bb_handle* h, const bb_score_opts* o, const bb_score_out* out);
// ... 21 lines not shown
    double* quantiles;
    int32_t* n_members;
    int32_t* n_steps;
} bb_theta_rb_out;
int bb_theta_rb_shape(const bb_handle* h, int64_t* n_groups);
int bb_theta_rb(bb_handle* h, const bb_rb_opts* o, const bb_theta_rb_out* out);

#define BB_POPMEAN_RB_CHUNK 256
typedef struct bb_popmean_rb_out {
    double *q_mean, *q_sd, *rb_mean, *rb_sd, *p_pos, *p_neg;
    double* quantiles;
    int32_t* n_members;
} bb_popmean_rb_out;
int bb_popmean_rb_shape(const bb_handle* h, int64_t* n_groups);
int bb_popmean_rb(bb_handle* h, const bb_rb_opts* o, const bb_popmean_rb_out* out);

#define BB_CHAIN_MAX_K 16384
#define BB_CHAIN_MAX_Q 8
#define BB_CHAIN_LAG_BATCH 32
#define BB_CHAIN_SLAB_BYTES (64 << 20)
typedef struct bb_chain_opts {
    int32_t n_chains;
    int32_t n_draws;
    int32_t n_quantiles;
    int32_t max_lag;
    const double* probs;
    int64_t slab_cols;
} bb_chain_opts;
typedef struct bb_chain_out {
    double *mean, *sd, *mcse, *ess, *rhat;
    double* quantiles;
    int32_t* n_lags;
} bb_chain_out;
int bb_chain_summary(bb_handle* h, const bb_chain_opts* o, int64_t n_cols,
                     const double* chain , const bb_chain_out* out);

#define BB_TRACE_MAX_SNAPSHOTS 16384
typedef struct bb_trace_opts {
    int32_t every;
    int32_t capacity;
} bb_trace_opts;
typedef struct bb_trace_sum_opts {
    int64_t first;
    int32_t n_chains;
    int32_t n_draws;
    int32_t max_lag;
    int32_t reserved0;
    int64_t slab_cols;
    double rhat_max;
} bb_trace_sum_opts;
typedef struct bb_trace_block {
    char name[24];
    int32_t part;
    int32_t reserved0;
    int64_t n_cols, n_nonfinite, n_const, n_above;
    double max_rhat, min_ess, max_mcse_rel;
} bb_trace_block;
typedef struct bb_trace_sum_out {
    double *mean, *sd, *mcse, *ess, *rhat;
    int32_t* n_lags;
    bb_trace_block* blocks;
} bb_trace_sum_out;
int bb_trace_begin(bb_handle* h, const bb_trace_opts* o);
int bb_trace_end(bb_handle* h);
int bb_trace_count(bb_handle* h, int64_t* taken, int64_t* first_live);
int bb_trace_get(bb_handle* h, int64_t first, int64_t n, double* mu , double* omega );
int bb_trace_summary(bb_handle* h, const bb_trace_sum_opts* o, const bb_trace_sum_out* out);

int bb_debug_normals(bb_handle* h, int64_t step, uint32_t stream, int64_t lo, int64_t hi, double* out);

#define BB_MATH_EXP 0
#define BB_MATH_LOG 1
#define BB_MATH_RCP 2
#define BB_MATH_DIV 3
#define BB_MATH_SQRT 4
#define BB_MATH_SOFTPLUS_SIGMOID 5
#define BB_MATH_SINCOSPI 6
#define BB_MATH_EXP_NONPOS 7
#define BB_MATH_LOG_1TO2 8
#define BB_MATH_BOX_MULLER 9
#define BB_MATH_COUNT 10
int bb_debug_math(bb_handle* h, int32_t fn, int64_t n, const double* x, const double* y, double* out0, double* out1);

int bb_debug_stamps(bb_handle* h, uint64_t* out, int64_t n);

int bb_debug_graph_launches(bb_handle* h);

int bb_get_stats(bb_handle* h, bb_stats* out);
int bb_kernel_name(bb_handle* h, char* buf, int64_t len);

#define BB_COMM_ID_BYTES 128
int bb_comm_make_id(void* id_out );
int bb_comm_init(bb_handle* h, const void* id );
int bb_step_moments(bb_handle* h, double* partial );
int bb_step_apply(bb_handle* h, const double* total );

#ifdef __cplusplus
}
#endif
#endif
```

Measured before the change: 70940.

## Add lean resident kernel variant and hoist per-wave facts out of the step loop

Result: no change. 71340, median of 6 (+0.6%).

```diff
diff --git a/barbay.jl_amd/_capi.py b/barbay.jl_amd/_capi.py
--- a/barbay.jl_amd/_capi.py
+++ b/barbay.jl_amd/_capi.py
@@ -32,7 +32,7 @@
 EXPORTS = [
     "bb_version", "bb_last_error", "bb_default_opts", "bb_create", "bb_destroy", "bb_num_latents",
     "bb_get_layout", "bb_init_meanfield", "bb_set_params", "bb_get_params", "bb_get_permutation", "bb_get_owned", "bb_run", "bb_run_profiled",
-    "bb_get_posterior", "bb_elbo_grad", "bb_logdensity_grad", "bb_logdensity_grad_batch", "bb_get_elbo_trace", "bb_debug_normals", "bb_debug_math", "bb_debug_stamps", "bb_debug_graph_launches", "bb_get_stats", "bb_kernel_name",
+    "bb_get_posterior", "bb_elbo_grad", "bb_logdensity_grad", "bb_logdensity_grad_batch", "bb_get_elbo_trace", "bb_debug_normals", "bb_debug_math", "bb_debug_opt_state", "bb_debug_stamps", "bb_debug_graph_launches", "bb_get_stats", "bb_kernel_name",
     "bb_comm_make_id", "bb_comm_init", "bb_step_moments", "bb_step_apply", "bb_hier_units", "bb_hier_fitness", "bb_p2p_export", "bb_p2p_import", "bb_p2p_selftest", "bb_p2p_enable",
     "bb_ppc_shape", "bb_ppc_bands", "bb_freq_shape", "bb_freq_bands", "bb_score_shape", "bb_ppc_score", "bb_chain_summary",
     "bb_fitness_rb_shape", "bb_fitness_rb", "bb_theta_rb_shape", "bb_theta_rb", "bb_popmean_rb_shape", "bb_popmean_rb",
@@ -82,7 +82,7 @@
         ("persistent_pairs", C.c_int32), ("launches_last_run", C.c_int32), ("resident_kernel", C.c_int32),
         ("geno_lo", C.c_int32), ("geno_hi", C.c_int32),
         ("device_bytes", C.c_int64), ("window_row", C.c_int64),
-        ("rows_same_xcd", C.c_int32), ("reserved0", C.c_int32),
+        ("rows_same_xcd", C.c_int32), ("lean_instance", C.c_int32),
     ]
 
 
@@ -211,6 +211,8 @@
     lib.bb_debug_normals.argtypes = [vp, C.c_int64, C.c_uint32, C.c_int64, C.c_int64, _dp]
     if hasattr(lib, "bb_debug_math"):
         lib.bb_debug_math.argtypes = [vp, C.c_int32, C.c_int64, _dp, _dp, _dp, _dp]
+    if hasattr(lib, "bb_debug_opt_state"):
+        lib.bb_debug_opt_state.argtypes = [vp, _dp, _dp, C.POINTER(C.c_float)]
     lib.bb_get_stats.argtypes = [vp, C.POINTER(bb_stats)]
     if hasattr(lib, "bb_kernel_name"):
         lib.bb_kernel_name.argtypes = [vp, C.c_char_p, C.c_int64]
@@ -456,6 +458,12 @@
                                             _ptr(out1) if out1 is not None else None))
         return out0, out1
 
+    def opt_state(self) -> Tuple[np.ndarray, np.ndarray, np.ndarray]:
+        D = self.D
+        am, ao, lo = np.empty(D), np.empty(D), np.empty((D, 2), dtype=np.float32)
+        self._check(self._lib.bb_debug_opt_state(self._h, _ptr(am), _ptr(ao), lo.ctypes.data_as(C.POINTER(C.c_float))))
+        return am, ao, lo
+
     def stamps(self, per_wave: bool = False) -> np.ndarray:
         nb = int(self.stats()["n_blocks"])
         rows = np.zeros(1, dtype=np.uint64)
diff --git a/barbay.jl_amd/csrc/bb_block.h b/barbay.jl_amd/csrc/bb_block.h
--- a/barbay.jl_amd/csrc/bb_block.h
+++ b/barbay.jl_amd/csrc/bb_block.h
@@ -344,14 +344,21 @@
     *s = t;
     *e = (a - (t - bb)) + (b - bb);
 }
+#if defined(BB_EMU)
+#define BB_PIN_VALUE(x) ((void)0)
+#else
+#define BB_PIN_VALUE(x) asm("" : "+v"(x))
+#endif
+template <bool LEAN = false>
 BB_DEV void bb_opt_apply(const DevModel& M, const DevState& S, const RunArgs& A, const BBSlot w,
                          int which, long long ih , double d, double old_slot, double* new_slot, double* p, double* acc, float* lo) {
     double upd;
-    if (A.opt == 0) {
-        const double n2 = d * d;
+    if (LEAN || A.opt == 0) {
+        double n2 = d * d;
+        if (LEAN) BB_PIN_VALUE(n2);
         *new_slot = n2;
         double s;
-        if (w.resum) {
+        if (!LEAN && w.resum) {
             s = 0.0;
             for (int j = 0; j < A.W; ++j) s += (j == w.slot) ? n2 : S.hist[((long long)j * 2 + which) * M.Dh + ih];
             *lo = 0.f;
@@ -367,6 +374,7 @@
         *acc = s;
         bb_cdouble* oc = bb_tab(S.optc);
         upd = d * (oc[0] * bb_rcp(oc[1] + bb_sqrt(s)));
+        if (LEAN) BB_PIN_VALUE(upd);
     } else {
         bb_cdouble* oc = bb_tab(S.optc);
         const double a = oc[3] * (*acc) + oc[2] * d * d;
diff --git a/barbay.jl_amd/csrc/bb_engine.hip b/barbay.jl_amd/csrc/bb_engine.hip
--- a/barbay.jl_amd/csrc/bb_engine.hip
+++ b/barbay.jl_amd/csrc/bb_engine.hip
@@ -47,6 +47,7 @@
     bool no_hist_pack, no_host_tables, no_res, no_persist, no_stream, force_stream, any_parity, force_allreduce, p2p_self;
     bool no_graph, graph_collective, no_regroup, no_reorder, nb_set, lead_set;
     int nb, res_nb, ng, lead, nthr, row_l2;
+    bool no_lean;
 };
 
 static BBTuning read_tuning() {
@@ -76,6 +77,7 @@
     if (t.lead < 10 || t.lead > 100) t.lead = 100;
     t.nthr = num("BB_TUNE_NTHR", 0) >= 64 ? num("BB_TUNE_NTHR", 0) / 64 * 64 : 0;
     t.row_l2 = num("BB_TUNE_ROW_L2", 1) == 0 ? 0 : 1;
+    t.no_lean = num("BB_TUNE_LEAN", 0) <= 0;
     return t;
 }
 
@@ -86,6 +88,7 @@
     int NB = 0, NBL = 0, nblk = 0;
     int ng = 8, pf = 0;
     bool ms = false;
+    bool lean = false;
     const void* fn = nullptr;
     std::string name;
     const char* why = nullptr;
@@ -304,6 +307,8 @@
             else if (MSrun) br_xchg_consume<KIND, PP, false, true>(cx, h->M, h->S, A, Y, sb, xc, &E.ok, want_el, ring, smp);
             else br_xchg_consume<KIND, PP, false, false>(cx, h->M, h->S, A, Y, sb, xc, &E.ok);
             if (MSrun) br_update<KIND, PP, 0, AP, true>(cx, h->M, h->S, A, Y, sb, wslot, buf, h->plan.NB, smp, NS);
+            else if (h->plan.lean && uniform_T(h->M) == 8) br_update<KIND, PP, 8, false, false, false, true>(cx, h->M, h->S, A, Y, sb, wslot, buf, h->plan.NB);
+            else if (h->plan.lean) br_update<KIND, PP, 6, false, false, false, true>(cx, h->M, h->S, A, Y, sb, wslot, buf, h->plan.NB);
             else if (!AP && uniform_T(h->M) == 8) br_update<KIND, PP, 8, false>(cx, h->M, h->S, A, Y, sb, wslot, buf, h->plan.NB);
             else if (!AP && uniform_T(h->M) == 6) br_update<KIND, PP, 6, false>(cx, h->M, h->S, A, Y, sb, wslot, buf, h->plan.NB);
             else br_update<KIND, PP, 0, AP>(cx, h->M, h->S, A, Y, sb, wslot, buf, h->plan.NB);
@@ -717,6 +722,16 @@
     return BB_OK;
 }
 
+extern "C" int bb_debug_opt_state(bb_handle* h, double* acc_mu, double* acc_omega, float* lo) {
+    if (!h || !acc_mu || !acc_omega || !lo) return bb_fail(BB_ERR_INVALID, "null argument");
+    BB_GROUP_UNSUPPORTED(h, "bb_debug_opt_state");
+    BB_ENTER(h);
+    int rc;
+    if ((rc = dsync(h->stream))) return rc;
+    if ((rc = d2h(acc_mu, h->S.acc_mu, (size_t)h->M.D * 8, h->stream)) || (rc = d2h(acc_omega, h->S.acc_om, (size_t)h->M.D * 8, h->stream))) return rc;
+    return d2h(lo, h->S.accl, (size_t)h->M.D * 2 * sizeof(float), h->stream);
+}
+
 static double host_softplus(double om) { return std::max(om, 0.0) + log1p(exp(-fabs(om))); }
 
 extern "C" int bb_get_posterior(bb_handle* h, double* mean, double* sigma) {
@@ -923,6 +938,7 @@
     s->persistent_pairs = h->plan.P;
     s->launches_last_run = h->launches_last_run;
     s->resident_kernel = h->plan.impl;
+    s->lean_instance = h->plan.lean ? 1 : 0;
     if (h->plan.impl >= IMPL_RES) {
         std::vector<int> sel((size_t)h->plan.nblk);
         int rc = d2h(sel.data(), h->S.xsel, sel.size() * sizeof(int), h->stream);
diff --git a/barbay.jl_amd/csrc/bb_inst.h b/barbay.jl_amd/csrc/bb_inst.h
--- a/barbay.jl_amd/csrc/bb_inst.h
+++ b/barbay.jl_amd/csrc/bb_inst.h
@@ -7,11 +7,11 @@
 typedef void (*bb_res_kernel)(const DevModel*, const DevState*, const BRLay*, RunArgs, int, int);
 #define BB_INST __attribute__((visibility("hidden")))
 BB_INST bb_persist_kernel bb_persist_instance(int kind, int P, int nthr, bool xg, const char** nm = nullptr);
-BB_INST bb_res_kernel bb_res_instance_k0(int P, int nthr, bool xg, int T, bool ap, bool ms, const char** nm = nullptr);
-BB_INST bb_res_kernel bb_res_instance_k1(int P, int nthr, bool xg, int T, bool ap, bool ms, const char** nm = nullptr);
-BB_INST bb_res_kernel bb_res_instance_k2(int P, int nthr, bool xg, int T, bool ap, bool ms, const char** nm = nullptr);
-BB_INST bb_res_kernel bb_res_instance_k3(int P, int nthr, bool xg, int T, bool ap, bool ms, const char** nm = nullptr);
-BB_INST bb_res_kernel bb_res_instance_k4(int P, int nthr, bool xg, int T, bool ap, bool ms, const char** nm = nullptr);
+BB_INST bb_res_kernel bb_res_instance_k0(int P, int nthr, bool xg, int T, bool ap, bool ms, const char** nm = nullptr, bool* lean = nullptr);
+BB_INST bb_res_kernel bb_res_instance_k1(int P, int nthr, bool xg, int T, bool ap, bool ms, const char** nm = nullptr, bool* lean = nullptr);
+BB_INST bb_res_kernel bb_res_instance_k2(int P, int nthr, bool xg, int T, bool ap, bool ms, const char** nm = nullptr, bool* lean = nullptr);
+BB_INST bb_res_kernel bb_res_instance_k3(int P, int nthr, bool xg, int T, bool ap, bool ms, const char** nm = nullptr, bool* lean = nullptr);
+BB_INST bb_res_kernel bb_res_instance_k4(int P, int nthr, bool xg, int T, bool ap, bool ms, const char** nm = nullptr, bool* lean = nullptr);
 BB_INST bb_stream_kernel bb_stream_instance(int kind, int nthr, int T, const char** nm = nullptr);
 BB_INST bb_stream_kernel bb_stream_instance_ms(int kind, int nthr, int T, const char** nm = nullptr);
 #endif
diff --git a/barbay.jl_amd/csrc/bb_inst_res.inc b/barbay.jl_amd/csrc/bb_inst_res.inc
--- a/barbay.jl_amd/csrc/bb_inst_res.inc
+++ b/barbay.jl_amd/csrc/bb_inst_res.inc
@@ -4,9 +4,13 @@
 #define BR_STR(x) BR_STR2(x)
 #define BR_NM(PP, NT, XG, TT, AP, MS) "k_res<" BR_STR(BR_K) "," #PP "," #NT "," XG "," #TT "," AP "," MS ">"
 #define BR_RET(PP, NT, XGb, XGs, TT, APb, APs, MSb, MSs) do { if (nm) *nm = BR_NM(PP, NT, XGs, TT, APs, MSs); return k_res<BR_K, PP, NT, XGb, TT, APb, MSb>; } while (0)
-bb_res_kernel BR_CAT(bb_res_instance_k, BR_K)(int P, int nthr, bool xg, int T, bool ap, bool ms, const char** nm) {
+#define BR_RETL(PP, NT, XGb, XGs, TT) do { if (nm) *nm = BR_NM(PP, NT, XGs, TT, "false", "false"); *lean = true; return k_res<BR_K, PP, NT, XGb, TT, false, false, true>; } while (0)
+bb_res_kernel BR_CAT(bb_res_instance_k, BR_K)(int P, int nthr, bool xg, int T, bool ap, bool ms, const char** nm, bool* lean) {
     if (nm) *nm = "";
-#define BR_T(PP, NT, TT) if (!ms && !ap && P == (PP) && T == (TT)) { if (xg) BR_RET(PP, NT, true, "true", TT, false, "false", false, "false"); BR_RET(PP, NT, false, "false", TT, false, "false", false, "false"); }
+    const bool want_lean = lean && *lean;
+    if (lean) *lean = false;
+#define BR_T(PP, NT, TT) if (!ms && !ap && P == (PP) && T == (TT)) { if (want_lean) { if (xg) BR_RETL(PP, NT, true, "true", TT); BR_RETL(PP, NT, false, "false", TT); } \
+                                                                     if (xg) BR_RET(PP, NT, true, "true", TT, false, "false", false, "false"); BR_RET(PP, NT, false, "false", TT, false, "false", false, "false"); }
 #define BR_CASE(PP, NT) case (PP): if (ms) { if (xg) { if (ap) BR_RET(PP, NT, true, "true", 0, true, "true", true, "true"); BR_RET(PP, NT, true, "true", 0, false, "false", true, "true"); } \
                                               if (ap) BR_RET(PP, NT, false, "false", 0, true, "true", true, "true"); BR_RET(PP, NT, false, "false", 0, false, "false", true, "true"); } \
                                   if (ap) { if (xg) BR_RET(PP, NT, true, "true", 0, true, "true", false, "false"); BR_RET(PP, NT, false, "false", 0, true, "true", false, "false"); } \
@@ -23,5 +27,6 @@
 #undef BR_T
 #undef BR_CASE
 #undef BR_RET
+#undef BR_RETL
 #undef BR_NM
 }
diff --git a/barbay.jl_amd/csrc/bb_plan.h b/barbay.jl_amd/csrc/bb_plan.h
--- a/barbay.jl_amd/csrc/bb_plan.h
+++ b/barbay.jl_amd/csrc/bb_plan.h
@@ -4,10 +4,13 @@
     return M.T[0];
 }
 
-static const void* resident_instance(const bb_handle* h, bool xg, bool stream, int P, bool ms, std::string& name) {
+static const void* resident_instance(const bb_handle* h, bool xg, bool stream, int P, bool ms, std::string& name, bool& lean) {
     const int kind = h->M.kind, nthr = h->nthr, T = uniform_T(h->M);
     const bool ap = br_any_parity(h->M);
+    const bool want_lean = lean && !stream;
+    lean = false;
 #if defined(BB_EMU)
+    lean = want_lean && !ms && !ap && (T == 8 || T == 6);
     char nm[64];
     if (stream) snprintf(nm, sizeof nm, "emu:k_stream<%d,%d,%d%s>", kind, nthr, T, ms ? ",true" : "");
     else snprintf(nm, sizeof nm, "emu:k_res<%d,%d,%d,%s,*,%s,%s>", kind, P, nthr, xg ? "true" : "false", ap ? "true" : "false", ms ? "true" : "false");
@@ -28,6 +31,8 @@
         if (nthr > 256 && nthr <= 512 && P == 3 && kind == 3) return fn(k_res<3, 3, 512, false, 0, true>);
         return nullptr;
     }
+    if (want_lean && nthr > 512 && P == 1 && kind == 0 && T == 8) { lean = true; return fn(k_res<0, 1, 1024, false, 8, false, false, true>); }
+    if (want_lean && nthr > 512 && P == 1 && kind == 1 && T == 6) { lean = true; return fn(k_res<1, 1, 1024, false, 6, false, false, true>); }
     if (nthr > 512 && P == 1 && kind == 0) return T == 8 ? fn(k_res<0, 1, 1024, false, 8>) : fn(k_res<0, 1, 1024, false>);
     if (nthr > 512 && P == 1 && kind == 1) return T == 6 ? fn(k_res<1, 1, 1024, false, 6>) : fn(k_res<1, 1, 1024, false>);
     if (nthr > 256 && nthr <= 512 && P == 2 && kind == 0) return T == 8 ? fn(k_res<0, 2, 512, false, 8>) : fn(k_res<0, 2, 512, false>);
@@ -38,15 +43,17 @@
 #else
     const char* nm = "";
     const void* k = nullptr;
+    bool got = want_lean;
     if (stream) k = ms ? (const void*)bb_stream_instance_ms(kind, nthr, T, &nm) : (const void*)bb_stream_instance(kind, nthr, T, &nm);
     else switch (kind) {
-        case 0: k = (const void*)bb_res_instance_k0(P, nthr, xg, T, ap, ms, &nm); break;
-        case 1: k = (const void*)bb_res_instance_k1(P, nthr, xg, T, ap, ms, &nm); break;
-        case 2: k = (const void*)bb_res_instance_k2(P, nthr, xg, T, ap, ms, &nm); break;
-        case 3: k = (const void*)bb_res_instance_k3(P, nthr, xg, T, ap, ms, &nm); break;
-        default: k = (const void*)bb_res_instance_k4(P, nthr, xg, T, ap, ms, &nm);
+        case 0: k = (const void*)bb_res_instance_k0(P, nthr, xg, T, ap, ms, &nm, &got); break;
+        case 1: k = (const void*)bb_res_instance_k1(P, nthr, xg, T, ap, ms, &nm, &got); break;
+        case 2: k = (const void*)bb_res_instance_k2(P, nthr, xg, T, ap, ms, &nm, &got); break;
+        case 3: k = (const void*)bb_res_instance_k3(P, nthr, xg, T, ap, ms, &nm, &got); break;
+        default: k = (const void*)bb_res_instance_k4(P, nthr, xg, T, ap, ms, &nm, &got);
     }
     name = nm;
+    lean = !stream && got;
     return k;
 #endif
 }
@@ -228,8 +235,12 @@
     return c.lds_doubles * 8 <= 160 * 1024;
 }
 
+static bool lean_wanted(const bb_handle* h, const LaunchPlan& p) {
+    return !h->tune.no_lean && p.impl == IMPL_RES && !p.ms && h->o.optimizer == BB_OPT_TRUNCATED_ADAGRAD && h->o.resum_every == 0 && p.pf == 1;
+}
 static bool instance_fits(const bb_handle* h, Planned& c) {
-    c.plan.fn = resident_instance(h, c.xg, c.plan.impl == IMPL_STREAM, c.plan.P, c.plan.ms, c.plan.name);
+    c.plan.lean = lean_wanted(h, c.plan);
+    c.plan.fn = resident_instance(h, c.xg, c.plan.impl == IMPL_STREAM, c.plan.P, c.plan.ms, c.plan.name, c.plan.lean);
     if (resident_fit(c.plan.fn, h->nthr, c.lds_doubles * 8, c.plan.nblk, h->cus)) return false;
     return c.plan.nblk <= h->tile_cap;
 }
diff --git a/barbay.jl_amd/csrc/bb_resident.h b/barbay.jl_amd/csrc/bb_resident.h
--- a/barbay.jl_amd/csrc/bb_resident.h
+++ b/barbay.jl_amd/csrc/bb_resident.h
@@ -180,6 +180,7 @@
     bb_d2 gp[P];
     bb_d2 gm[P], go[P];
     double el;
+    bb_d2 ep[P], sp[P], sg[P];
 };
 
 enum { BRM_A0 = 1 << 4, BRM_A1 = 1 << 5, BRM_VALID = 1 << 6, BRM_MUT = 1 << 7, BRM_PREV = 1 << 8, BRM_NEXT = 1 << 9 };
@@ -538,6 +539,11 @@
     if (KIND <= 1) return kind == SK_LS_E ? 1 : -1;
     return kind == SK_LT_R ? 1 : (kind == SK_LS_R ? 2 : -1);
 }
+template <int KIND> BB_DEV bool br_needs_exp(int meta) {
+    const int kd = meta & 15;
+    return (meta & BRM_VALID) && (kd == SK_L || (kd < SK_GS && br_stage_trn<KIND>(kd) >= 0));
+}
+BB_DEV bool br_holds_unit(int meta) { return (meta & BRM_VALID) && (meta & 15) != SK_L; }
 template <int KIND>
 BB_DEV void br_unit_sw(const double* lds, const BRLay& Y, int buf, int o, int thoff, double* s, double* w) {
     const double* b = lds + buf * Y.SU;
@@ -553,8 +559,14 @@
 template <int P, bool HD = false>
 BB_DEV void br_prefetch_slot(BBCtx& cx, const DevModel& M, const DevState& S, const RunArgs& A, const BRLay& Y, BRSt<P>* stv, int slot);
 template <int KIND, int P> BB_DEV void br_pair_prior(const double* lds, const BRLay& Y, const BRSt<P>& st, int k, bool a0, bool a1, double* pm0, double* iv0, double* pm1, double* iv1);
+#ifdef BR_NO_PRE_AH
+template <int KIND, int P> BB_DEV constexpr bool br_pre_ah() { return false; }
+#else
+template <int KIND, int P> BB_DEV constexpr bool br_pre_ah() { return P == 1 && KIND <= 1; }
+#endif
+enum { BRW_EXP = 1, BRW_UNIT = 2 };
 template <int KIND, int P, bool MS = false, bool HD = false>
-BB_DEV void br_sample(BBCtx& cx, const DevModel& M, const DevState& S, const RunArgs& A, const BRLay& Y, BRSt<P>* stv, int buf, int slot, bool prefetch = true, bool want_el = false) {
+BB_DEV void br_sample(BBCtx& cx, const DevModel& M, const DevState& S, const RunArgs& A, const BRLay& Y, BRSt<P>* stv, int buf, int slot, bool prefetch = true, bool want_el = false, int wf = -1) {
     double* lds = cx.lds;
     const BBLds& L = Y.L;
     BB_STAMP(cx, S, 20);
@@ -574,8 +586,11 @@
             bb_softplus_sigmoid(st.om[k].x, &sp0, &sg0);
             bb_softplus_sigmoid(st.om[k].y, &sp1, &sg1);
             st.z[k] = bb_d2{fma(sp0, e.x, st.mu[k].x), fma(sp1, e.y, st.mu[k].y)};
-            st.a[k] = bb_d2{e.x * sg0, e.y * sg1};
-            st.h[k] = bb_d2{sg0 * bb_rcp(sp0), sg1 * bb_rcp(sp1)};
+            if (br_pre_ah<KIND, P>()) { st.ep[k] = e; st.sp[k] = bb_d2{sp0, sp1}; st.sg[k] = bb_d2{sg0, sg1}; }
+            else {
+                st.a[k] = bb_d2{e.x * sg0, e.y * sg1};
+                st.h[k] = bb_d2{sg0 * bb_rcp(sp0), sg1 * bb_rcp(sp1)};
+            }
             if (MS && want_el) {
                 if (k == 0) st.el = 0.0;
                 const int meta = st.meta[k], kd = meta & 15;
@@ -592,7 +607,7 @@
             const int kd = st.meta[k] & 15;
             const double f = (kd == SK_LS_E || (KIND >= 2 && kd == SK_LS_R)) ? -2.0 : 1.0;
 #ifndef BB_EMU
-            if (__builtin_amdgcn_ballot_w64((st.meta[k] & BRM_VALID) && (kd == SK_L || (kd < SK_GS && br_stage_trn<KIND>(kd) >= 0))) == 0ull) st.lam[k] = bb_d2{0.0, 0.0};
+            if (wf >= 0 ? !(wf & BRW_EXP) : __builtin_amdgcn_ballot_w64((st.meta[k] & BRM_VALID) && (kd == SK_L || (kd < SK_GS && br_stage_trn<KIND>(kd) >= 0))) == 0ull) st.lam[k] = bb_d2{0.0, 0.0};
             else
 #endif
             st.lam[k] = bb_d2{bb_exp(f * st.z[k].x), bb_exp(f * st.z[k].y)};
@@ -904,6 +919,13 @@
 #pragma unroll
         for (int k = 0; k < P; ++k) {
             const int meta = st.meta[k];
+            if (br_pre_ah<KIND, P>()) {
+                st.a[k] = bb_d2{st.ep[k].x * st.sg[k].x, st.ep[k].y * st.sg[k].y};
+                st.h[k] = bb_d2{st.sg[k].x * bb_rcp(st.sp[k].x), st.sg[k].y * bb_rcp(st.sp[k].y)};
+#ifndef BB_EMU
+                asm volatile("" : "+v"(st.a[k].x), "+v"(st.a[k].y), "+v"(st.h[k].x), "+v"(st.h[k].y));
+#endif
+            }
             if ((meta & 15) != SK_L || !(meta & BRM_VALID)) continue;
             const bool hp = meta & BRM_PREV, hn = meta & BRM_NEXT;
             double pm0, iv0, pm1, iv1, z0, z1, ap, am, an, wp, wm, wn;
@@ -1016,18 +1038,21 @@
     *g1 = fma(st.lam[k].y, lds[Y.iG + pt + 1], st.gp[k].y) + (rn - rm);
 }
 
-template <int KIND, int P, int TT = 0, bool AP = false, bool MS = false, bool HD = false>
+template <int KIND, int P, int TT = 0, bool AP = false, bool MS = false, bool HD = false, bool LEAN = false>
 BB_DEV void br_update(BBCtx& cx, const DevModel& M, const DevState& S, const RunArgs& A, const BRLay& Y, BRSt<P>* stv,
-                      const BBSlot wslot, int buf, int NBs, int smp = 0, int NS = 1) {
+                      const BBSlot wslot, int buf, int NBs, int smp = 0, int NS = 1, int wf = -1) {
     double* lds = cx.lds;
     const BBLds& L = Y.L;
     BB_STAMP_WAVE(cx, S, A, 2);
 #ifndef BB_EMU
     {
-        bool u = false;
-#pragma unroll
-        for (int k = 0; k < P; ++k) u = u || ((stv->meta[k] & BRM_VALID) && (stv->meta[k] & 15) != SK_L);
-        if (__builtin_amdgcn_ballot_w64(u) != 0ull) __builtin_amdgcn_s_setprio(3);
+        if (wf >= 0) { if (wf & BRW_UNIT) __builtin_amdgcn_s_setprio(3); }
+        else {
+            bool u = false;
+#pragma unroll
+            for (int k = 0; k < P; ++k) u = u || ((stv->meta[k] & BRM_VALID) && (stv->meta[k] & 15) != SK_L);
+            if (__builtin_amdgcn_ballot_w64(u) != 0ull) __builtin_amdgcn_s_setprio(3);
+        }
     }
 #endif
     const double* zbuf = lds + Y.zl + buf * Y.NBT;
@@ -1035,7 +1060,7 @@
         BRSt<P>& st = BB_PSTATE(stv, tid);
         double* hs_m = nullptr;
         double* hs_o = nullptr;
-        if (A.opt == 0) {
+        if (LEAN || A.opt == 0) {
             hs_m = S.hist + ((long long)wslot.slot * 2 + 0) * M.Dh;
             hs_o = S.hist + ((long long)wslot.slot * 2 + 1) * M.Dh;
         }
@@ -1141,7 +1166,7 @@
                 go0 = go0 * invS + st.h[k].x; go1 = go1 * invS + st.h[k].y;
             } else { go0 = fma(g0, st.a[k].x, st.h[k].x); go1 = fma(g1, st.a[k].y, st.h[k].y); }
             bb_d2 hm{0, 0}, ho{0, 0};
-            if (hs_m) {
+            if (LEAN || hs_m) {
 #ifndef BB_EMU
                 asm volatile("s_waitcnt vmcnt(0)" ::: "memory");
 #endif
@@ -1151,18 +1176,18 @@
             bb_d2 nhm = hm, nho = ho;
             const long long ih = st.i0[k] - BR_HDELTA(HD, lds, Y, meta);
             if (a0) {
-                bb_opt_apply(M, S, A, wslot, 0, ih, -g0, hm.x, &nhm.x, &st.mu[k].x, &st.am[k].x, &st.lo[k].x);
+                bb_opt_apply<LEAN>(M, S, A, wslot, 0, ih, -g0, hm.x, &nhm.x, &st.mu[k].x, &st.am[k].x, &st.lo[k].x);
                 BR_SCHED_FENCE();
-                bb_opt_apply(M, S, A, wslot, 1, ih, -go0, ho.x, &nho.x, &st.om[k].x, &st.ao[k].x, &st.lo[k].y);
+                bb_opt_apply<LEAN>(M, S, A, wslot, 1, ih, -go0, ho.x, &nho.x, &st.om[k].x, &st.ao[k].x, &st.lo[k].y);
                 BR_SCHED_FENCE();
             }
             if (a1) {
-                bb_opt_apply(M, S, A, wslot, 0, ih + 1, -g1, hm.y, &nhm.y, &st.mu[k].y, &st.am[k].y, &st.lo[k].z);
+                bb_opt_apply<LEAN>(M, S, A, wslot, 0, ih + 1, -g1, hm.y, &nhm.y, &st.mu[k].y, &st.am[k].y, &st.lo[k].z);
                 BR_SCHED_FENCE();
-                bb_opt_apply(M, S, A, wslot, 1, ih + 1, -go1, ho.y, &nho.y, &st.om[k].y, &st.ao[k].y, &st.lo[k].w);
+                bb_opt_apply<LEAN>(M, S, A, wslot, 1, ih + 1, -go1, ho.y, &nho.y, &st.om[k].y, &st.ao[k].y, &st.lo[k].w);
                 BR_SCHED_FENCE();
             }
-            if (hs_m) { br_store_pair_stream<AP>(hs_m, ih, a0, a1, nhm); br_store_pair_stream<AP>(hs_o, ih, a0, a1, nho); }
+            if (LEAN || hs_m) { br_store_pair_stream<AP>(hs_m, ih, a0, a1, nhm); br_store_pair_stream<AP>(hs_o, ih, a0, a1, nho); }
         }
     }
 #ifndef BB_EMU
@@ -1221,7 +1246,7 @@
 }
 
 #ifndef BB_EMU
-template <int KIND, int P, int NT, bool XG = false, int TT = 0, bool AP = false, bool MS = false>
+template <int KIND, int P, int NT, bool XG = false, int TT = 0, bool AP = false, bool MS = false, bool LEAN = false>
 __global__ void __launch_bounds__(NT) k_res(const DevModel* __restrict__ Mp, const DevState* __restrict__ Sp, const BRLay* __restrict__ Yp,
                                             RunArgs A, int NB, int nsteps) {
     const DevModel& M = *Mp;
@@ -1230,6 +1255,7 @@
     extern __shared__ __attribute__((aligned(16))) double br_smem[];
     BBCtx cx{(int)blockDim.x, (int)blockIdx.x, br_smem, nullptr};
     BRSt<P> st;
+    if (LEAN) { A.opt = 0; A.resum_every = 0; A.pf = 1; }
     int* ok_slot = (int*)(br_smem + Yp->L.misc) + 1;
     const unsigned long long c0 = S.ctr[0], c1 = S.ctr[1];
     unsigned long long step0 = c0 > c1 ? c0 : c1;
@@ -1239,6 +1265,12 @@
     BB_STAMP_RT(cx, S, 3);
     const bool dead = *ok_slot == 0;
     int done = 0;
+    int wf = -1;
+#ifndef BR_NO_WAVE_FACTS
+    if (P == 1 && KIND <= 1)
+        wf = __builtin_amdgcn_readfirstlane((__builtin_amdgcn_ballot_w64(br_needs_exp<KIND>(st.meta[0])) != 0ull ? BRW_EXP : 0) |
+                                            (__builtin_amdgcn_ballot_w64(br_holds_unit(st.meta[0])) != 0ull ? BRW_UNIT : 0));
+#endif
     if (!dead) {
         br_draw_ahead<KIND, P, AP>(cx, A, Y, &st, step0);
         BB_STAMP_RT(cx, S, 4);
@@ -1259,13 +1291,13 @@
 #pragma unroll
                     for (int k = 0; k < P; ++k) asm volatile("" : "+v"(st.meta[k]));
                 }
-                br_sample<KIND, P, MS, XG>(cx, M, S, A, Y, &st, buf, wslot.slot, last, want_el);
+                br_sample<KIND, P, MS, XG>(cx, M, S, A, Y, &st, buf, wslot.slot, last, want_el, wf);
                 br_moments<KIND, P, MS>(cx, M, S, Y, &st, buf, A.xepoch0 + (unsigned)(xc + 1), want_el);
                 br_xchg_publish<KIND, P, AP, XG>(cx, M, S, A, Y, &st, xc, wslot.slot, last ? step + 1 : step, last ? 0u : (unsigned)(smp + 1), last);
                 br_xchg_lead<XG>(cx, M, S, A, Y, xc, ok_slot);
                 br_xchg_consume<KIND, P, XG, MS>(cx, M, S, A, Y, &st, xc, ok_slot, want_el, ring, smp);
                 if (*ok_slot == 0) { stop = true; break; }
-                br_update<KIND, P, TT, AP, MS, XG>(cx, M, S, A, Y, &st, wslot, buf, NB, smp, NS);
+                br_update<KIND, P, TT, AP, MS, XG, LEAN>(cx, M, S, A, Y, &st, wslot, buf, NB, smp, NS, wf);
             }
             if (stop) break;
             if (MS && A.elbo_every > 0) {
diff --git a/include/barbay_hip.h b/include/barbay_hip.h
--- a/include/barbay_hip.h
+++ b/include/barbay_hip.h
@@ -99,7 +99,7 @@
     int64_t device_bytes;
     int64_t window_row;
     int32_t rows_same_xcd;
-    int32_t reserved0;
+    int32_t lean_instance;
 } bb_stats;
 
 const char* bb_version(void);
@@ -287,6 +287,8 @@
 #define BB_MATH_COUNT 10
 int bb_debug_math(bb_handle* h, int32_t fn, int64_t n, const double* x, const double* y, double* out0, double* out1);
 
+int bb_debug_opt_state(bb_handle* h, double* acc_mu, double* acc_omega, float* lo);
+
 int bb_debug_stamps(bb_handle* h, uint64_t* out, int64_t n);
 
 int bb_debug_graph_launches(bb_handle* h);
```
